# zcablii/SM3Det

Measured on NVIDIA H100. Metric: backbone images/sec @1024^2 (fwd+bwd), higher is better.
Workload: dtype f32 (bf16 hi+lo split operands on wgmma, fp32 accumulate; SIMT fp32 elsewhere)

## Files before the change

include/sm3det_b200.h:

```cpp
#ifndef SM3DET_B200_H_
#define SM3DET_B200_H_

#include <stddef.h>
#include <stdint.h>

#ifdef __cplusplus
extern "C" {
#endif

#define SM3_ABI_VERSION 1

#define SM3_OK 0
#define SM3_ERR_INVALID_ARG (-1)
#define SM3_ERR_UNSUPPORTED_SHAPE (-2)
#define SM3_ERR_CUDA (-3)
#define SM3_ERR_WORKSPACE (-4)

int sm3_abi_version(void);
const char* sm3_last_error(void);
int sm3_device_supported(void);

enum { SM3_SCHED_DENSE = 0, SM3_SCHED_GROUPED = 1, SM3_SCHED_SPLITK = 2 };
enum {
  SM3_EPI_BIAS = 1,
  SM3_EPI_GELU = 2,
  SM3_EPI_DGELU = 4,
  SM3_EPI_COLSCALE = 8,
  SM3_EPI_ROWSCALE = 16,
  SM3_EPI_RESID = 32,
  SM3_EPI_ATOMIC = 64,
  SM3_EPI_AUXSTORE = 128,
  SM3_EPI_COLSUM = 256
};
typedef struct sm3_gemm_args {
  const float* A; int64_t a_stride_mn, a_stride_k;
  const float* B; int64_t b_stride_mn, b_stride_k, b_group_stride;
  const int32_t* a_row_index;
  const int32_t* b_k_index;
  const uint16_t* b_packed;
  int64_t b_packed_group_stride;
  const uint16_t* a_packed;
  int32_t M, N, K;
  int32_t tile_n;
  int32_t sched;
  int32_t k_splits, num_groups;
  const int32_t* tile_group;
  const int32_t* num_m_tiles;
  const int32_t* seg_begin;
  const int32_t* seg_end;
  float* D; int64_t ldd, d_group_stride;
  const float* bias; int64_t bias_group_stride;
  int32_t epilogue;
  float* aux_out; const float* aux_in; int64_t ld_aux;
  const float* col_scale; const float* row_scale;
  const float* resid; int64_t ld_resid;
  float* colsum; int64_t colsum_group_stride;
  int32_t mma_passes;
} sm3_gemm_args;
int sm3_gemm(const sm3_gemm_args* args, void* stream);
int64_t sm3_gemm_packed_elems(int32_t N, int32_t K);
int sm3_gemm_pack_b(const float* B, int64_t stride_mn, int64_t stride_k, int64_t group_stride, int32_t groups,
                    int32_t N, int32_t K, uint16_t* out, void* stream);
int64_t sm3_gemm_packed_act_elems(int64_t rows, int32_t cols, int32_t mn_major, int32_t tile);
int sm3_gemm_pack_act(const float* X, int64_t ld, const int32_t* row_index, int64_t rows, int32_t cols,
                      int32_t mn_major, int32_t tile, uint16_t* out, void* stream);
int32_t sm3_gemm_tile_n(int32_t N);
int sm3_gemm_pack_b_tile(const float* B, int64_t stride_mn, int64_t stride_k, int64_t group_stride, int32_t groups,
                         int32_t N, int32_t K, int32_t tile, uint16_t* out, void* stream);
size_t sm3_gemm_workspace_bytes(const sm3_gemm_args* args);

typedef struct sm3_ffn_args {
  const uint16_t* a1; const uint16_t* a2;
  const uint16_t* wa1; const uint16_t* wa2; const uint16_t* wb;
  const float* bias1;
  const float* bias2;
  const float* col_scale;
  const float* row_scale;
  const float* resid;
  float* out;
  float* aux_out;
  float* h_out;
  int32_t M, C, H4, chunk, mma_passes, mode;
} sm3_ffn_args;
int32_t sm3_ffn_fused_chunk(int32_t mode, int32_t C);
int sm3_ffn_fused(const sm3_ffn_args* args, void* stream);
size_t sm3_ffn_fused_workspace_bytes(const sm3_ffn_args* args);

enum { SM3_LN_NHWC = 0, SM3_LN_PATCH2 = 1, SM3_LN_NCHW = 2 };
int sm3_layernorm_fwd(const float* x, const float* weight, const float* bias, float* y, float* stats,
                      int64_t tokens, int32_t C, float eps, int32_t out_mode, int32_t H, int32_t W, void* stream);
int sm3_layernorm_fwd_img(const float* x, const float* weight, const float* bias, uint16_t* img, float* y, float* stats,
                          int64_t T, int32_t C, float eps, void* stream);
int sm3_layernorm_bwd(const float* dy, const float* x, const float* stats, const float* weight, float* dx,
                      float* dweight, float* dbias, int64_t tokens, int32_t C, int32_t in_mode, int32_t H,
                      int32_t W, int32_t dx_accumulate, void* stream);

int sm3_stem_fwd(const float* x_nchw, const float* weight_t, const float* bias, const float* ln_weight,
                 const float* ln_bias, float* y, float* conv_out, float* stats, int32_t N, int32_t Cin,
                 int32_t H, int32_t W, int32_t ps, int32_t C0, float eps, void* stream);
int sm3_stem_wgrad(const float* x_nchw, const float* dconv, float* dweight_t, float* dbias, int32_t N,
                   int32_t Cin, int32_t H, int32_t W, int32_t ps, int32_t C0, void* stream);

int sm3_dwconv7_fwd(const float* x, const float* weight_t, const float* bias, const float* resid, float* y,
                    int32_t N, int32_t H, int32_t W, int32_t C, void* stream);
int sm3_dwconv7_wgrad(const float* x, const float* dy, float* dweight_t, float* dbias, int32_t N, int32_t H,
                      int32_t W, int32_t C, void* stream);

typedef struct sm3_router_args {
  const float* v; const float* proj_weight; const float* proj_bias; const float* sim_matrix;
  const float* temperature; const float* w_noise; const float* noise;
  int32_t T, C, P, E, k;
  int32_t* top_idx; float* top_gate; float* logits; float* top_vals; float* p_out;
  float* sigma; int32_t* top_idx_m;
  float* partials;
} sm3_router_args;
int sm3_moe_router_blocks(int32_t T);
int sm3_moe_router(const sm3_router_args* args, void* stream);
size_t sm3_moe_router_workspace_bytes(const sm3_router_args* args);

typedef struct sm3_plan_args {
  const float* partials; int32_t T, E, k, max_m_tiles;
  float* importance; float* load; float* loss;
  int32_t* counts; int32_t* seg_begin; int32_t* seg_end; int32_t* cursor;
  int32_t* tile_group; int32_t* num_m_tiles;
} sm3_plan_args;
int sm3_moe_plan(const sm3_plan_args* args, void* stream);
size_t sm3_moe_plan_workspace_bytes(const sm3_plan_args* args);
int sm3_moe_assign(const int32_t* top_idx, int32_t T, int32_t k, int32_t E, const int32_t* seg_begin,
                   int32_t* cursor, int32_t* slot_of, int32_t* pair_token, void* stream);
int sm3_moe_combine(const float* expert_out, const int32_t* slot_of, const int32_t* top_idx, const float* gate,
                    const float* gamma, const float* resid, const float* row_scale, float* out, float* y_opt,
                    int32_t T, int32_t C, int32_t k, void* stream);

typedef struct sm3_act_pack_args {
  const float* h; const float* da; int64_t R; int32_t W; int32_t mode;
  const int32_t* live_tiles; const int32_t* tile_group;
  float* out_f32; uint16_t* pack_k; uint16_t* pack_mn; int32_t mn_tile; float* colsum;
  uint16_t* pack_mn2; int32_t mn_tile2;
} sm3_act_pack_args;
int sm3_act_pack(const sm3_act_pack_args* args, void* stream);

int sm3_moe_combine_bwd(const float* dout, const float* expert_out, const int32_t* slot_of, const int32_t* top_idx,
                        const float* gate, const float* gamma, const float* row_scale, float* d_expert_out,
                        float* dgate, float* dgamma, int32_t T, int32_t C, int32_t k, void* stream);
typedef struct sm3_router_bwd_args {
  const float* p; const float* sim_matrix; const float* temperature;
  const int32_t* top_idx; const float* top_gate; const float* dgate; const float* logits;
  const float* importance; const float* loss_scale;
  int32_t T, P, E, k;
  float* dp; float* dsim_hat; float* dtemperature;
  const float* noise; const float* sigma; const float* top_vals; const int32_t* top_idx_m; const float* load;
  float* dr;
} sm3_router_bwd_args;
int sm3_moe_router_bwd(const sm3_router_bwd_args* args, void* stream);
int sm3_moe_router_bwd_finalize(const float* dsim_hat, const float* sim_matrix, float* dsim, int32_t P, int32_t E,
                                void* stream);
int sm3_colsum(const float* a, const float* b, const float* row_scale, const int32_t* seg_begin,
               const int32_t* seg_end, int32_t groups, float* out, int64_t rows, int32_t C, void* stream);
int sm3_gather_sum(const float* src, const int32_t* slot_of, const float* add, float* out, int32_t T, int32_t C,
                   int32_t k, void* stream);
int sm3_scale_rows(const float* x, const float* row_scale, const float* col_scale, float* out, int64_t rows,
                   int32_t C, void* stream);

int sm3_gather_rows_peer(const float* const* bases, const int32_t* const* token_lists, const int32_t* src_rank,
                         const int32_t* src_row, const float* scale, float* out, int64_t rows, int32_t C, void* stream);

typedef struct sm3_ep_plan_args {
  const int32_t* allm; const int32_t* tile_group_s; const int32_t* num_tiles_s; const int32_t* pair_token;
  int32_t W, me, E, R_s, cap;
  int32_t* src_rank; int32_t* src_slot; int32_t* tile_group; int32_t* num_tiles; int32_t* seg_begin; int32_t* seg_end;
  int32_t* comb_rank; int32_t* comb_row; int32_t* overflow;
} sm3_ep_plan_args;
int sm3_ep_plan(const sm3_ep_plan_args* args, void* stream);

int sm3_dwconv_fwd(const float* x, const float* weight_t, const float* bias, const float* resid, float* y, int32_t N,
                   int32_t H, int32_t W, int32_t C, int32_t ks, int32_t dil, void* stream);
int sm3_dwconv_wgrad(const float* x, const float* dy, float* dweight_t, float* dbias, int32_t N, int32_t H, int32_t W,
                     int32_t C, int32_t ks, int32_t dil, void* stream);
int sm3_colstat(const float* x, const float* sh1, const float* y, const float* sh2, const float* sc2, float* s1, float* s2,
                int64_t rows, int32_t C, void* stream);
int sm3_affine(const float* x1, const float* a1, const float* x2, const float* a2, const float* b, const float* add,
               float* out, int64_t rows, int32_t C, void* stream);
int sm3_mul(const float* a, const float* b, const float* add, float* out, int64_t n, void* stream);
int sm3_dropout(const float* x, float* out, int64_t n, float p, uint64_t seed, void* stream);
int sm3_dropout_dev(const float* x, float* out, int64_t n, float p, const uint64_t* seed_dev, void* stream);
int sm3_lsk_agg(const float* a1, const float* a2, float* agg, int32_t* amax, int64_t T, int32_t Ch, void* stream);
int sm3_conv7_c2(const float* x, const float* w, const float* b, float* y, int32_t N, int32_t H, int32_t W, int32_t act,
                 void* stream);
int sm3_conv7_c2_wgrad(const float* x, const float* dpre, float* dw, float* db, int32_t N, int32_t H, int32_t W, void* stream);
int sm3_lsk_mix(const float* a1, const float* a2, const float* sig, float* out, int64_t T, int32_t Ch, void* stream);
int sm3_lsk_mix_bwd_sig(const float* dout, const float* a1, const float* a2, const float* sig, float* dpre, int64_t T,
                        int32_t Ch, void* stream);
int sm3_lsk_mix_bwd_in(const float* dout, const float* sig, const float* dagg, const int32_t* amax, float* da1, float* da2,
                       int64_t T, int32_t Ch, void* stream);
int sm3_im2col(const float* x, float* col, int32_t N, int32_t H, int32_t W, int32_t Cin, int32_t ks, int32_t stride,
               int32_t pad, int32_t Kp, int32_t nchw, void* stream);
int sm3_col2im(const float* dcol, float* dx, int32_t N, int32_t H, int32_t W, int32_t Cin, int32_t ks, int32_t stride,
               int32_t pad, int32_t Kp, int32_t nchw, void* stream);

int sm3_upsample_add(const float* a, const float* b, float* out, int32_t N, int32_t H, int32_t W, int32_t h, int32_t w,
                     int32_t C, void* stream);
int sm3_upsample_add_bwd(const float* d, float* db, int32_t N, int32_t H, int32_t W, int32_t h, int32_t w, int32_t C,
                         void* stream);
int sm3_transpose_batched(const float* in, float* out, int32_t B, int32_t R, int32_t Cc, void* stream);

#ifdef __cplusplus
}
#endif
#endif
```

sm3det_b200/_lib.py:

```python
import ctypes as C
import os
import threading

_LIB_PATH = os.path.join(os.path.dirname(os.path.abspath(__file__)), 'lib', 'libsm3det_b200.so')
_lock = threading.Lock()
_lib = None
LAUNCHES = 0

c_f32p = C.c_void_p
c_i32p = C.c_void_p
c_stream = C.c_void_p


class GemmArgs(C.Structure):
    _fields_ = [
        ('A', c_f32p), ('a_stride_mn', C.c_int64), ('a_stride_k', C.c_int64),
        ('B', c_f32p), ('b_stride_mn', C.c_int64), ('b_stride_k', C.c_int64), ('b_group_stride', C.c_int64),
        ('a_row_index', c_i32p), ('b_k_index', c_i32p), ('b_packed', C.c_void_p), ('b_packed_group_stride', C.c_int64), ('a_packed', C.c_void_p),
        ('M', C.c_int32), ('N', C.c_int32), ('K', C.c_int32),
        ('tile_n', C.c_int32), ('sched', C.c_int32), ('k_splits', C.c_int32), ('num_groups', C.c_int32),
        ('tile_group', c_i32p), ('num_m_tiles', c_i32p), ('seg_begin', c_i32p), ('seg_end', c_i32p),
        ('D', c_f32p), ('ldd', C.c_int64), ('d_group_stride', C.c_int64),
        ('bias', c_f32p), ('bias_group_stride', C.c_int64),
        ('epilogue', C.c_int32),
        ('aux_out', c_f32p), ('aux_in', c_f32p), ('ld_aux', C.c_int64),
        ('col_scale', c_f32p), ('row_scale', c_f32p),
        ('resid', c_f32p), ('ld_resid', C.c_int64),
        ('colsum', c_f32p), ('colsum_group_stride', C.c_int64),
        ('mma_passes', C.c_int32),
    ]


class RouterArgs(C.Structure):
    _fields_ = [
        ('v', c_f32p), ('proj_weight', c_f32p), ('proj_bias', c_f32p), ('sim_matrix', c_f32p),
        ('temperature', c_f32p), ('w_noise', c_f32p), ('noise', c_f32p),
        ('T', C.c_int32), ('C', C.c_int32), ('P', C.c_int32), ('E', C.c_int32), ('k', C.c_int32),
        ('top_idx', c_i32p), ('top_gate', c_f32p), ('logits', c_f32p), ('top_vals', c_f32p), ('p_out', c_f32p),
        ('sigma', c_f32p), ('top_idx_m', c_i32p),
        ('partials', c_f32p),
    ]


class PlanArgs(C.Structure):
    _fields_ = [
        ('partials', c_f32p), ('T', C.c_int32), ('E', C.c_int32), ('k', C.c_int32), ('max_m_tiles', C.c_int32),
        ('importance', c_f32p), ('load', c_f32p), ('loss', c_f32p),
        ('counts', c_i32p), ('seg_begin', c_i32p), ('seg_end', c_i32p), ('cursor', c_i32p),
        ('tile_group', c_i32p), ('num_m_tiles', c_i32p),
    ]


class FfnArgs(C.Structure):
    _fields_ = [
        ('a1', C.c_void_p), ('a2', C.c_void_p), ('wa1', C.c_void_p), ('wa2', C.c_void_p), ('wb', C.c_void_p),
        ('bias1', c_f32p), ('bias2', c_f32p), ('col_scale', c_f32p), ('row_scale', c_f32p), ('resid', c_f32p),
        ('out', c_f32p), ('aux_out', c_f32p), ('h_out', c_f32p),
        ('M', C.c_int32), ('C', C.c_int32), ('H4', C.c_int32), ('chunk', C.c_int32), ('mma_passes', C.c_int32),
        ('mode', C.c_int32),
    ]


class EpPlanArgs(C.Structure):
    _fields_ = [
        ('allm', c_i32p), ('tile_group_s', c_i32p), ('num_tiles_s', c_i32p), ('pair_token', c_i32p),
        ('W', C.c_int32), ('me', C.c_int32), ('E', C.c_int32), ('R_s', C.c_int32), ('cap', C.c_int32),
        ('src_rank', c_i32p), ('src_slot', c_i32p), ('tile_group', c_i32p), ('num_tiles', c_i32p),
        ('seg_begin', c_i32p), ('seg_end', c_i32p), ('comb_rank', c_i32p), ('comb_row', c_i32p), ('overflow', c_i32p),
    ]


_I32, _I64, _F32, _P = C.c_int32, C.c_int64, C.c_float, C.c_void_p
SIGNATURES = {
    'sm3_abi_version': [],
    'sm3_last_error': [],
    'sm3_device_supported': [],
    'sm3_gemm': [C.POINTER(GemmArgs), _P],
    'sm3_gemm_packed_elems': [_I32, _I32],
    'sm3_gemm_pack_b': [_P, _I64, _I64, _I64, _I32, _I32, _I32, _P, _P],
    'sm3_gemm_packed_act_elems': [_I64, _I32, _I32, _I32],
    'sm3_gemm_pack_act': [_P, _I64, _P, _I64, _I32, _I32, _I32, _P, _P],
    'sm3_gemm_tile_n': [_I32],
    'sm3_gemm_pack_b_tile': [_P, _I64, _I64, _I64, _I32, _I32, _I32, _I32, _P, _P],
    'sm3_gemm_workspace_bytes': [C.POINTER(GemmArgs)],
    'sm3_ffn_fused_chunk': [_I32, _I32],
    'sm3_ffn_fused': [C.POINTER(FfnArgs), _P],
    'sm3_ffn_fused_workspace_bytes': [C.POINTER(FfnArgs)],
    'sm3_moe_router_workspace_bytes': [C.POINTER(RouterArgs)],
    'sm3_moe_plan_workspace_bytes': [C.POINTER(PlanArgs)],
    'sm3_layernorm_fwd': [_P, _P, _P, _P, _P, _I64, _I32, _F32, _I32, _I32, _I32, _P],
    'sm3_layernorm_fwd_img': [_P, _P, _P, _P, _P, _P, _I64, _I32, _F32, _P],
    'sm3_layernorm_bwd': [_P, _P, _P, _P, _P, _P, _P, _I64, _I32, _I32, _I32, _I32, _I32, _P],
    'sm3_stem_fwd': [_P, _P, _P, _P, _P, _P, _P, _P, _I32, _I32, _I32, _I32, _I32, _I32, _F32, _P],
    'sm3_stem_wgrad': [_P, _P, _P, _P, _I32, _I32, _I32, _I32, _I32, _I32, _P],
    'sm3_dwconv7_fwd': [_P, _P, _P, _P, _P, _I32, _I32, _I32, _I32, _P],
    'sm3_dwconv7_wgrad': [_P, _P, _P, _P, _I32, _I32, _I32, _I32, _P],
    'sm3_moe_router_bwd_finalize': [_P, _P, _P, _I32, _I32, _P],
    'sm3_moe_router_blocks': [_I32],
    'sm3_moe_router': [C.POINTER(RouterArgs), _P],
    'sm3_moe_plan': [C.POINTER(PlanArgs), _P],
    'sm3_moe_assign': [_P, _I32, _I32, _I32, _P, _P, _P, _P, _P],
    'sm3_moe_combine': [_P, _P, _P, _P, _P, _P, _P, _P, _P, _I32, _I32, _I32, _P],
    'sm3_moe_combine_bwd': [_P, _P, _P, _P, _P, _P, _P, _P, _P, _P, _I32, _I32, _I32, _P],
    'sm3_colsum': [_P, _P, _P, _P, _P, _I32, _P, _I64, _I32, _P],
    'sm3_gather_sum': [_P, _P, _P, _P, _I32, _I32, _I32, _P],
    'sm3_scale_rows': [_P, _P, _P, _P, _I64, _I32, _P],
    'sm3_moe_router_bwd': [_P, _P],
    'sm3_ep_plan': [C.POINTER(EpPlanArgs), _P],
    'sm3_gather_rows_peer': [_P, _P, _P, _P, _P, _P, _I64, _I32, _P],
    'sm3_upsample_add': [_P, _P, _P, _I32, _I32, _I32, _I32, _I32, _I32, _P],
    'sm3_upsample_add_bwd': [_P, _P, _I32, _I32, _I32, _I32, _I32, _I32, _P],
    'sm3_transpose_batched': [_P, _P, _I32, _I32, _I32, _P],
    'sm3_dwconv_fwd': [_P, _P, _P, _P, _P, _I32, _I32, _I32, _I32, _I32, _I32, _P],
    'sm3_dwconv_wgrad': [_P, _P, _P, _P, _I32, _I32, _I32, _I32, _I32, _I32, _P],
    'sm3_colstat': [_P, _P, _P, _P, _P, _P, _P, _I64, _I32, _P],
    'sm3_affine': [_P, _P, _P, _P, _P, _P, _P, _I64, _I32, _P],
    'sm3_mul': [_P, _P, _P, _P, _I64, _P],
    'sm3_dropout': [_P, _P, _I64, _F32, C.c_uint64, _P],
    'sm3_dropout_dev': [_P, _P, _I64, _F32, _P, _P],
    'sm3_lsk_agg': [_P, _P, _P, _P, _I64, _I32, _P],
    'sm3_conv7_c2': [_P, _P, _P, _P, _I32, _I32, _I32, _I32, _P],
    'sm3_conv7_c2_wgrad': [_P, _P, _P, _P, _I32, _I32, _I32, _P],
    'sm3_lsk_mix': [_P, _P, _P, _P, _I64, _I32, _P],
    'sm3_lsk_mix_bwd_sig': [_P, _P, _P, _P, _P, _I64, _I32, _P],
    'sm3_lsk_mix_bwd_in': [_P, _P, _P, _P, _P, _P, _I64, _I32, _P],
    'sm3_im2col': [_P, _P, _I32, _I32, _I32, _I32, _I32, _I32, _I32, _I32, _I32, _P],
    'sm3_col2im': [_P, _P, _I32, _I32, _I32, _I32, _I32, _I32, _I32, _I32, _I32, _P],
}
_RESTYPES = {'sm3_last_error': C.c_char_p, 'sm3_gemm_packed_elems': C.c_int64, 'sm3_gemm_packed_act_elems': C.c_int64,
             'sm3_gemm_workspace_bytes': C.c_size_t, 'sm3_ffn_fused_workspace_bytes': C.c_size_t,
             'sm3_moe_router_workspace_bytes': C.c_size_t, 'sm3_moe_plan_workspace_bytes': C.c_size_t}


class ActPackArgs(C.Structure):
    _fields_ = [
        ('h', c_f32p), ('da', c_f32p), ('R', C.c_int64), ('W', C.c_int32), ('mode', C.c_int32),
        ('live_tiles', c_i32p), ('tile_group', c_i32p),
        ('out_f32', c_f32p), ('pack_k', C.c_void_p), ('pack_mn', C.c_void_p), ('mn_tile', C.c_int32), ('colsum', c_f32p),
        ('pack_mn2', C.c_void_p), ('mn_tile2', C.c_int32),
    ]


class RouterBwdArgs(C.Structure):
    _fields_ = [
        ('p', c_f32p), ('sim_matrix', c_f32p), ('temperature', c_f32p),
        ('top_idx', c_i32p), ('top_gate', c_f32p), ('dgate', c_f32p), ('logits', c_f32p),
        ('importance', c_f32p), ('loss_scale', c_f32p),
        ('T', C.c_int32), ('P', C.c_int32), ('E', C.c_int32), ('k', C.c_int32),
        ('dp', c_f32p), ('dsim_hat', c_f32p), ('dtemperature', c_f32p),
        ('noise', c_f32p), ('sigma', c_f32p), ('top_vals', c_f32p), ('top_idx_m', c_i32p), ('load', c_f32p),
        ('dr', c_f32p),
    ]


SIGNATURES['sm3_moe_router_bwd'] = [C.POINTER(RouterBwdArgs), _P]
SIGNATURES['sm3_act_pack'] = [C.POINTER(ActPackArgs), _P]


def library_path() -> str:
    return _LIB_PATH


def load():
    global _lib
    if _lib is not None:
        return _lib
    with _lock:
        if _lib is not None:
            return _lib
        if not os.path.isfile(_LIB_PATH):
            raise RuntimeError(
                f'sm3det_b200: CUDA library not built ({_LIB_PATH} missing). Run `make` at the repo root or '
                f'`python -c "import __graft_entry__ as g; g.build()"`. There is no CPU/PyTorch fallback.')
        lib = C.CDLL(_LIB_PATH)
        for name, argtypes in SIGNATURES.items():
            fn = getattr(lib, name)
            fn.argtypes = argtypes
            fn.restype = _RESTYPES.get(name, C.c_int)
        if lib.sm3_abi_version() != 1:
            raise RuntimeError('sm3det_b200: ABI version mismatch')
        _lib = lib
    return _lib


def check(rc: int, what: str):
    global LAUNCHES
    LAUNCHES += 1
    if rc != 0:
        msg = load().sm3_last_error()
        raise RuntimeError(f'sm3det_b200: {what} failed (rc={rc}): {msg.decode() if msg else "?"}')
```

sm3det_b200/backbone.py:

```python
import math
from typing import Sequence

import torch
import torch.nn as nn

from . import functional as Fn
from .registry import ROTATED_BACKBONES, BaseModule

ARCH_SETTINGS = {
    'atto': dict(depths=[2, 2, 6, 2], channels=[40, 80, 160, 320]),
    'femto': dict(depths=[2, 2, 6, 2], channels=[48, 96, 192, 384]),
    'pico': dict(depths=[2, 2, 6, 2], channels=[64, 128, 256, 512]),
    'nano': dict(depths=[2, 2, 8, 2], channels=[80, 160, 320, 640]),
    'tiny': dict(depths=[3, 3, 9, 3], channels=[96, 192, 384, 768]),
    'small': dict(depths=[3, 3, 27, 3], channels=[96, 192, 384, 768]),
    'base': dict(depths=[3, 3, 27, 3], channels=[128, 256, 512, 1024]),
    'swin_large': dict(depths=[2, 2, 18, 2], channels=[192, 384, 768, 1536]),
    'large': dict(depths=[3, 3, 27, 3], channels=[192, 384, 768, 1536]),
    'xlarge': dict(depths=[3, 3, 27, 3], channels=[256, 512, 1024, 2048]),
    'huge': dict(depths=[3, 3, 27, 3], channels=[352, 704, 1408, 2816]),
}


class LayerNorm2d(nn.LayerNorm):

    def __init__(self, num_channels: int, **kwargs) -> None:
        super().__init__(num_channels, **kwargs)
        self.num_channels = self.normalized_shape[0]


def build_LayerNorm2d_layer(cfg: dict, num_features: int) -> nn.Module:
    if not isinstance(cfg, dict):
        raise TypeError('cfg must be a dict')
    if 'type' not in cfg:
        raise KeyError('the cfg dict must contain the key "type"')
    cfg_ = cfg.copy()
    cfg_.pop('type')
    requires_grad = cfg_.pop('requires_grad', True)
    cfg_.setdefault('eps', 1e-5)
    layer = LayerNorm2d(num_features, **cfg_)
    for param in layer.parameters():
        param.requires_grad = requires_grad
    return layer


class FFN(nn.Module):
    def __init__(self, in_channels, mid_channels):
        super().__init__()
        self.pointwise_conv1 = nn.Linear(in_channels, mid_channels)
        self.pointwise_conv2 = nn.Linear(mid_channels, in_channels)


class CosineTopKGate(nn.Module):
    def __init__(self, model_dim, num_global_experts, init_t=0.5):
        super().__init__()
        proj_dim = min(model_dim // 2, 256)
        self.temperature = nn.Parameter(torch.log(torch.full([1], 1.0 / init_t)), requires_grad=True)
        self.cosine_projector = nn.Linear(model_dim, proj_dim)
        self.sim_matrix = nn.Parameter(torch.randn(size=(proj_dim, num_global_experts)), requires_grad=True)
        nn.init.normal_(self.sim_matrix, 0, 0.01)


class MoE_layer(nn.Module):
    def __init__(self, in_channels, mid_channels, num_experts, top_k, noisy_gating, gating):
        super().__init__()
        if gating != 'cosine':
            raise NotImplementedError(
                "sm3det_b200: only gate='cosine' is implemented (gate='linear' starts from an all-zero w_gate, "
                'i.e. fully tied logits whose routing is implementation-defined in the reference)')
        assert top_k <= num_experts
        self.noisy_gating = noisy_gating
        self.num_experts = num_experts
        self.input_size = in_channels
        self.k = top_k
        self.gating = gating
        self.experts = nn.ModuleList([FFN(in_channels, mid_channels) for _ in range(num_experts)])
        self.w_gate = CosineTopKGate(in_channels, num_experts)
        self.w_noise = nn.Parameter(torch.zeros(in_channels, num_experts), requires_grad=True)
        self.register_buffer('mean', torch.tensor([0.0]))
        self.register_buffer('std', torch.tensor([1.0]))

    def expert_params(self):
        e = self.experts
        w1 = [m.pointwise_conv1.weight for m in e]
        b1 = [m.pointwise_conv1.bias for m in e]
        w2 = [m.pointwise_conv2.weight for m in e]
        b2 = [m.pointwise_conv2.bias for m in e]
        for group in (w1, b1, w2, b2):
            Fn.stack_expert_params(group)
        return w1 + b1 + w2 + b2


class PackCache:

    def __init__(self):
        self._d = {}

    def invalidate(self):
        self._d.clear()

    def get(self, name, params, transposed, tile=0):
        from . import ops
        key = tuple(p._version for p in params) + (params[0].data_ptr(), str(params[0].device))
        name = (name, tile)
        hit = self._d.get((name, transposed))
        if hit is not None and hit[0] == key:
            return hit[1]
        reuse = None if hit is None or hit[1][0].device != params[0].device else hit[1][0]
        with torch.no_grad():
            packed = ops.pack_weight(params[0], transposed=transposed, groups=len(params), out=reuse, tile=tile)
        self._d[(name, transposed)] = (key, packed)
        return packed


class ConvNeXtBlock(nn.Module):
    def __init__(self, in_channels, norm_cfg, mlp_ratio=4., MoE_cfg=None, drop_path_rate=0.,
                 layer_scale_init_value=1e-6):
        super().__init__()
        self.depthwise_conv = nn.Conv2d(in_channels, in_channels, groups=in_channels, kernel_size=7, padding=3)
        self.norm = build_LayerNorm2d_layer(norm_cfg, in_channels)
        mid = int(mlp_ratio * in_channels)
        self.MoE_cfg = MoE_cfg
        if MoE_cfg is not None:
            self.ffn = MoE_layer(in_channels, mid, MoE_cfg['num_experts'], MoE_cfg['top_k'], MoE_cfg['noisy_gating'],
                                 MoE_cfg['gating'])
        else:
            self.ffn = FFN(in_channels, mid)
        if not layer_scale_init_value > 0:
            raise NotImplementedError('sm3det_b200: layer_scale_init_value must be > 0 (gamma is fused in the epilogue)')
        self.gamma = nn.Parameter(layer_scale_init_value * torch.ones((in_channels)), requires_grad=True)
        self.drop_path_rate = float(drop_path_rate)
        self._packs = PackCache()

    def _apply(self, fn, recurse=True):
        self._packs.invalidate()
        return super()._apply(fn, recurse)

    def _load_from_state_dict(self, *args, **kwargs):
        self._packs.invalidate()
        return super()._load_from_state_dict(*args, **kwargs)

    def _row_scale(self, x):
        if self.drop_path_rate == 0. or not self.training:
            return None
        keep = 1.0 - self.drop_path_rate
        N, H, W, _ = x.shape
        mask = getattr(self, '_injected_drop_mask', None)
        if mask is None:
            mask = x.new_empty((N,)).bernoulli_(keep)
            if keep > 0.0:
                mask = mask / keep
        return mask.to(x.device, torch.float32).repeat_interleave(H * W).contiguous()

    def forward(self, x, record=None):
        return self._run(x, self._row_scale(x), record, True)

    def _run(self, x, rs, record, shortcut):
        eps = self.norm.eps
        dw = self.depthwise_conv
        grad = torch.is_grad_enabled()
        pc = self._packs
        from . import ops
        if self.MoE_cfg is None:
            f = self.ffn
            w1, w2 = f.pointwise_conv1.weight, f.pointwise_conv2.weight
            C = w2.shape[0]
            cf = ops.ffn_chunk(0, C)
            if cf > 0:
                packs = {'fused': dict(fwd=cf), 'w1_c': pc.get('w1', [w1], False, tile=cf), 'w2_n': pc.get('w2', [w2], False, tile=C)}
            else:
                packs = {'w1': pc.get('w1', [w1], False), 'w2': pc.get('w2', [w2], False)}
            if grad:
                packs['w1_t'] = pc.get('w1', [w1], True)
            packs['grad'] = grad
            packs['shortcut'] = shortcut
            out = Fn.DenseBlockFn.apply(x, dw.weight, dw.bias, self.norm.weight, self.norm.bias,
                                        w1, f.pointwise_conv1.bias, w2, f.pointwise_conv2.bias, self.gamma, rs, eps, packs)
            return out, None
        m = self.ffn
        noise = None
        if m.noisy_gating and self.training:
            noise = getattr(m, '_injected_noise', None)
            if noise is None:
                T = x.shape[0] * x.shape[1] * x.shape[2]
                noise = torch.randn((T, m.num_experts), device=x.device, dtype=torch.float32)
            noise = noise.to(x.device, torch.float32).contiguous()
        g = m.w_gate
        ep = m.expert_params()
        E = m.num_experts
        w1s, w2s = ep[0:E], ep[2 * E:3 * E]
        epc = getattr(self, '_ep', None)
        if epc is not None:
            if not shortcut:
                raise NotImplementedError('sm3det_b200: expert parallelism is not wired for the ConvNeXt_DA blocks')
            from .expert_parallel import EPMoEBlockFn
            El = E // epc.world
            o1, o2 = w1s[epc.rank * El:(epc.rank + 1) * El], w2s[epc.rank * El:(epc.rank + 1) * El]
            packs = {'w1': pc.get('w1', o1, False), 'w2': pc.get('w2', o2, False)}
            if grad:
                packs['w1_t'] = pc.get('w1', o1, True)
                packs['w2_t'] = pc.get('w2', o2, True)
                packs['wp_t'] = pc.get('wp', [g.cosine_projector.weight], True)
            return EPMoEBlockFn.apply(x, dw.weight, dw.bias, self.norm.weight, self.norm.bias, self.gamma,
                                      g.cosine_projector.weight, g.cosine_projector.bias, g.sim_matrix, g.temperature,
                                      m.w_noise, rs, noise, eps, E, m.k, record, packs, epc, self._ep_key, *ep)
        packs = {'w1': pc.get('w1', w1s, False), 'w2': pc.get('w2', w2s, False)}
        if grad:
            packs['w1_t'] = pc.get('w1', w1s, True)
            packs['w2_t'] = pc.get('w2', w2s, True)
            packs['wp_t'] = pc.get('wp', [g.cosine_projector.weight], True)
        packs['shortcut'] = shortcut
        out, loss = Fn.MoEBlockFn.apply(x, dw.weight, dw.bias, self.norm.weight, self.norm.bias, self.gamma,
                                        g.cosine_projector.weight, g.cosine_projector.bias, g.sim_matrix, g.temperature,
                                        m.w_noise, rs, noise, eps, E, m.k, record, packs, *ep)
        return out, loss


class DALayer(nn.Module):
    dataset_DA = {'sar': 0, 'rgb': 1, 'ifr': 2}

    def __init__(self, channel, reduction=16):
        super().__init__()
        self.avg_pool = nn.AdaptiveAvgPool2d(1)
        self.fc = nn.ModuleList([nn.Sequential(nn.Linear(channel, channel // reduction, bias=False), nn.ReLU(inplace=True),
                                               nn.Linear(channel // reduction, channel, bias=False), nn.Sigmoid())] * 3)

    def gate(self, m, datasets):
        with torch.autocast('cuda', enabled=False):
            if len(datasets) == 1:
                return self.fc[self.dataset_DA[datasets[0]]](m)
            if len(datasets) != m.shape[0]:
                raise ValueError(f'ConvNeXt_DA: {len(datasets)} dataset names for a batch of {m.shape[0]} (the reference zips them '
                                 f'sample by sample, convnext_moe_DA.py:315-318)')
            return torch.cat([self.fc[self.dataset_DA[d]](row.view(1, -1)) for row, d in zip(m, datasets)], dim=0)


class ConvNeXtDABlock(ConvNeXtBlock):

    def __init__(self, *args, **kwargs):
        super().__init__(*args, **kwargs)
        self.avg_pool = nn.AdaptiveAvgPool2d(1)
        self.DA = DALayer(self.gamma.shape[0])

    def forward(self, x, record=None, datasets=('rgb',)):
        rs = self._row_scale(x)
        y, loss = self._run(x, None, record, False)
        s = self.DA.gate(Fn.SampleMeanFn.apply(y), list(datasets))
        return Fn.DAGateFn.apply(y, x, s, rs), loss


@ROTATED_BACKBONES.register_module()
class ConvNeXt_moe(BaseModule):
    arch_settings = ARCH_SETTINGS
    block_cls = ConvNeXtBlock

    def __init__(self, arch='tiny', in_channels=3, stem_patch_size=4, norm_cfg=dict(type='LN2d', eps=1e-6),
                 act_cfg=dict(type='GELU'), linear_pw_conv=True, use_grn=False, drop_path_rate=0.,
                 layer_scale_init_value=1e-6, out_indices=[0, 1, 2, 3], MoE_Block_inds=[[], [], [], []],
                 noisy_gating=True, num_experts=2, gate='cosine', top_k=2, frozen_stages=0,
                 gap_before_final_norm=False, with_cp=False,
                 init_cfg=[dict(type='TruncNormal', layer=['Conv2d', 'Linear'], std=.02, bias=0.),
                           dict(type='Constant', layer=['LayerNorm'], val=1., bias=0.)]):
        super().__init__(init_cfg=init_cfg)
        if isinstance(arch, str):
            assert arch in self.arch_settings, \
                f'Unavailable arch, please choose from ({set(self.arch_settings)}) or pass a dict.'
            arch = self.arch_settings[arch]
        elif isinstance(arch, dict):
            assert 'depths' in arch and 'channels' in arch, \
                f'The arch dict must have "depths" and "channels", but got {list(arch.keys())}.'
        if act_cfg.get('type', 'GELU') != 'GELU':
            raise NotImplementedError('sm3det_b200: only act_cfg=dict(type="GELU") is implemented')
        if not linear_pw_conv:
            raise NotImplementedError('sm3det_b200: linear_pw_conv=False (1x1 Conv2d FFN) is not implemented')
        if use_grn:
            raise NotImplementedError('sm3det_b200: use_grn=True is not implemented (no SM3Det config enables it)')
        if gap_before_final_norm:
            raise NotImplementedError('sm3det_b200: gap_before_final_norm=True is not implemented')
        self.depths = list(arch['depths'])
        self.channels = list(arch['channels'])
        assert (isinstance(self.depths, Sequence) and isinstance(self.channels, Sequence)
                and len(self.depths) == len(self.channels))
        for c in self.channels:
            if c % 32 != 0 or c > 1024:
                raise NotImplementedError(f'sm3det_b200: channel count {c} unsupported (multiple of 32, <= 1024)')
        self.num_stages = len(self.depths)
        if isinstance(out_indices, int):
            out_indices = [out_indices]
        out_indices = list(out_indices)
        for i, index in enumerate(out_indices):
            if index < 0:
                out_indices[i] = 4 + index
                assert out_indices[i] >= 0, f'Invalid out_indices {index}'
        self.out_indices = out_indices
        self.MoE_Block_inds = MoE_Block_inds
        self.num_experts = num_experts
        self.frozen_stages = frozen_stages
        self.gap_before_final_norm = gap_before_final_norm
        self.with_cp = with_cp
        self.stem_patch_size = stem_patch_size
        self.norm_eps = norm_cfg.get('eps', 1e-5)

        dpr = [x.item() for x in torch.linspace(0, drop_path_rate, sum(self.depths), device='cpu')]
        block_idx = 0
        self.downsample_layers = nn.ModuleList()
        stem = nn.Sequential(
            nn.Conv2d(in_channels, self.channels[0], kernel_size=stem_patch_size, stride=stem_patch_size),
            build_LayerNorm2d_layer(norm_cfg, self.channels[0]))
        self.downsample_layers.append(stem)
        self.stages = nn.ModuleList()
        for i in range(self.num_stages):
            depth = self.depths[i]
            channels = self.channels[i]
            if i >= 1:
                self.downsample_layers.append(nn.Sequential(
                    build_LayerNorm2d_layer(norm_cfg, self.channels[i - 1]),
                    nn.Conv2d(self.channels[i - 1], channels, kernel_size=2, stride=2)))
            moe_ind = [list(range(depth))[q] for q in self.MoE_Block_inds[i] if q < depth]
            stage = nn.Sequential(*[
                self.block_cls(in_channels=channels, drop_path_rate=dpr[block_idx + j], norm_cfg=norm_cfg,
                              MoE_cfg={'noisy_gating': noisy_gating, 'num_experts': num_experts, 'top_k': top_k,
                                       'gating': gate} if j in moe_ind else None,
                              layer_scale_init_value=layer_scale_init_value) for j in range(depth)])
            block_idx += depth
            self.stages.append(stage)
            if i in self.out_indices:
                self.add_module(f'norm{i}', build_LayerNorm2d_layer(norm_cfg, channels))
        self._init_like_reference()
        self._freeze_stages()

    def _init_like_reference(self):
        """The reference never runs init_cfg (init_weights() only supports 'Pretrained'); weights stay at
        torch defaults.  We keep torch's default constructors too, so nothing to do."""

    def _stem(self, x):
        conv, ln = self.downsample_layers[0][0], self.downsample_layers[0][1]
        return Fn.StemFn.apply(x, conv.weight, conv.bias, ln.weight, ln.bias, ln.eps, self.stem_patch_size)

    def _trunk(self, x, record=None, datasets=None):
        outs, gate_losses = [], []
        for i, stage in enumerate(self.stages):
            if i >= 1:
                ln, conv = self.downsample_layers[i][0], self.downsample_layers[i][1]
                x = Fn.DownsampleFn.apply(x, ln.weight, ln.bias, conv.weight, conv.bias, ln.eps)
            for blk in stage:
                x, gate_loss = blk(x, record) if datasets is None else blk(x, record, datasets)
                if gate_loss is not None:
                    gate_losses.append(gate_loss)
            if i in self.out_indices:
                nl = getattr(self, f'norm{i}')
                outs.append(Fn.OutNormFn.apply(x, nl.weight, nl.bias, nl.eps))
        if len(gate_losses) > 0:
            return tuple(outs), sum(gate_losses) / len(gate_losses)
        return tuple(outs)

    def forward(self, x, record=None):
        self._check_input(x)
        with self._precision():
            return self._trunk(self._stem(x), record)

    def _precision(self):
        from . import ops
        return ops.precision_scope(ops.autocast_passes(self))

    @staticmethod
    def _check_input(x):
        if not x.is_cuda:
            raise RuntimeError('sm3det_b200 backbones run on CUDA (sm_90a) only; there is no CPU path')
        if x.dim() != 4 or x.shape[2] % 32 != 0 or x.shape[3] % 32 != 0:
            raise ValueError(f'expected [N,3,H,W] with H, W multiples of 32 (Pad size_divisor=32), got {tuple(x.shape)}')

    def _freeze_stages(self):
        for i in range(self.frozen_stages):
            downsample_layer = self.downsample_layers[i]
            stage = self.stages[i]
            downsample_layer.eval()
            stage.eval()
            for param in list(downsample_layer.parameters()) + list(stage.parameters()):
                param.requires_grad = False

    def train(self, mode=True):
        super().train(mode)
        self._freeze_stages()
        return self

    def get_layer_depth(self, param_name: str, prefix: str = ''):
        max_layer_id = 12 if self.depths[-2] > 9 else 6
        if not param_name.startswith(prefix):
            return max_layer_id + 1, max_layer_id + 2
        param_name = param_name[len(prefix):]
        if param_name.startswith('downsample_layers'):
            stage_id = int(param_name.split('.')[1])
            if stage_id == 0:
                layer_id = 0
            elif stage_id == 1 or stage_id == 2:
                layer_id = stage_id + 1
            else:
                layer_id = max_layer_id
        elif param_name.startswith('stages'):
            stage_id = int(param_name.split('.')[1])
            block_id = int(param_name.split('.')[2])
            if stage_id == 0 or stage_id == 1:
                layer_id = stage_id + 1
            elif stage_id == 2:
                layer_id = 3 + block_id // 3
            else:
                layer_id = max_layer_id
        else:
            layer_id = max_layer_id + 1
        return layer_id, max_layer_id + 2

    def upcycle_state_dict(self, src, multi_input=False):
        out = {}
        for k, v in src.items():
            if not k.startswith('backbone.'):
                continue
            k = k[9:]
            if multi_input and 'downsample_layers.0.0' in k:
                out[k.replace('downsample_layers.0.0', 'dataset_stems.single')] = v
            elif multi_input and 'downsample_layers.0.1' in k:
                out[k.replace('downsample_layers.0.1', 'downsample_layers.0.0')] = v
            elif 'pointwise_conv' in k:
                parts = k.split('.')
                stage_ind, block_ind = int(parts[1]), int(parts[2])
                if block_ind in self.MoE_Block_inds[stage_ind]:
                    for e in range(self.num_experts):
                        out[k.replace('pointwise_conv', f'ffn.experts.{e}.pointwise_conv')] = v
                else:
                    out[k.replace('pointwise_conv', 'ffn.pointwise_conv')] = v
            else:
                out[k] = v
        if out and next(iter(out)).startswith('module.'):
            out = {k[7:]: v for k, v in out.items()}
        return out

    def init_weights(self):
        cfg = self.init_cfg
        if isinstance(cfg, dict) and cfg.get('type') == 'Pretrained' and cfg.get('checkpoint'):
            ckpt = torch.load(cfg['checkpoint'], map_location='cpu')
            sd = ckpt.get('state_dict', ckpt.get('model', ckpt))
            sd = self.upcycle_state_dict(sd, multi_input=isinstance(self, ConvNeXt_moe_MultiInput))
            print(self.load_state_dict(sd, strict=False))


@ROTATED_BACKBONES.register_module()
class ConvNeXt_moe_MultiInput(ConvNeXt_moe):
    def __init__(self, arch='tiny', in_channels=3, stem_patch_size=4, datasets=None,
                 norm_cfg=dict(type='LN2d', eps=1e-6), act_cfg=dict(type='GELU'), linear_pw_conv=True,
                 use_grn=False, drop_path_rate=0., layer_scale_init_value=1e-6, out_indices=[0, 1, 2, 3],
                 MoE_Block_inds=[[], [], [], []], noisy_gating=True, num_experts=2, top_k=2, gate='cosine',
                 frozen_stages=0, gap_before_final_norm=False, with_cp=False,
                 init_cfg=[dict(type='TruncNormal', layer=['Conv2d', 'Linear'], std=.02, bias=0.),
                           dict(type='Constant', layer=['LayerNorm'], val=1., bias=0.)]):
        super().__init__(MoE_Block_inds=MoE_Block_inds, noisy_gating=noisy_gating, num_experts=num_experts,
                         gate=gate, top_k=top_k, arch=arch, in_channels=in_channels,
                         stem_patch_size=stem_patch_size, norm_cfg=norm_cfg, act_cfg=act_cfg,
                         linear_pw_conv=linear_pw_conv, use_grn=use_grn, drop_path_rate=drop_path_rate,
                         layer_scale_init_value=layer_scale_init_value, out_indices=out_indices,
                         frozen_stages=frozen_stages, gap_before_final_norm=gap_before_final_norm,
                         with_cp=with_cp, init_cfg=init_cfg)
        self.downsample_layers[0] = nn.Sequential(build_LayerNorm2d_layer(norm_cfg, self.channels[0]))
        self.datasets = ['single']
        self.dataset_stems = nn.ModuleDict()
        self.dataset_stems['single'] = nn.Conv2d(in_channels, self.channels[0], kernel_size=stem_patch_size,
                                                 stride=stem_patch_size)

    def _stem(self, x):
        conv, ln = self.dataset_stems['single'], self.downsample_layers[0][0]
        return Fn.StemFn.apply(x, conv.weight, conv.bias, ln.weight, ln.bias, ln.eps, self.stem_patch_size)

    def forward(self, x, datasets=['single'], record=None):
        if len(datasets) == 1:
            x = [x]
        x = torch.cat(list(x), dim=0)
        self._check_input(x)
        with self._precision():
            return self._trunk(self._stem(x), record)


@ROTATED_BACKBONES.register_module()
class ConvNeXt_DA_MultiInput(ConvNeXt_moe_MultiInput):
    block_cls = ConvNeXtDABlock

    def __init__(self, *args, datasets=None, **kwargs):
        super().__init__(*args, datasets=datasets, **kwargs)
        if datasets is not None and list(datasets) != ['single']:
            raise NotImplementedError('sm3det_b200: per-dataset stems (datasets=[...]) are not implemented; the reference forward '
                                      "only ever uses dataset_stems['single'] (convnext_moe_DA.py:836)")
        self.init_datasets = datasets

    def forward(self, x, datasets=['single'], record=None):
        if len(datasets) == 1:
            x = [x]
        x = torch.cat(list(x), dim=0)
        self._check_input(x)
        with self._precision():
            return self._trunk(self._stem(x), record, list(datasets))

    def init_weights(self):
        super().init_weights()
        cfg = self.init_cfg
        if isinstance(cfg, dict) and cfg.get('type') == 'Pretrained':
            for stage in self.stages:
                for blk in stage:
                    for m in range(3):
                        nn.init.constant_(blk.DA.fc[m][2].weight, 0.0)
```

sm3det_b200/csrc/capi.cu:

```cuda
#include "../../include/sm3det_b200.h"
#include "common.cuh"
#include "gemm_tc.cuh"
#include "kernels.h"
#include "ffn_fused.cuh"

using namespace sm3;

static inline cudaStream_t S(void* s) { return reinterpret_cast<cudaStream_t>(s); }

extern "C" {

int sm3_abi_version(void) { return SM3_ABI_VERSION; }
const char* sm3_last_error(void) { return sm3::last_error(); }

int sm3_device_supported(void) {
  int dev = 0, major = 0, minor = 0;
  if (cudaGetDevice(&dev) != cudaSuccess) return 0;
  if (cudaDeviceGetAttribute(&major, cudaDevAttrComputeCapabilityMajor, dev) != cudaSuccess) return 0;
  if (cudaDeviceGetAttribute(&minor, cudaDevAttrComputeCapabilityMinor, dev) != cudaSuccess) return 0;
  return (major == 9 && minor == 0) ? 1 : 0;
}

int sm3_gemm(const sm3_gemm_args* a, void* stream) {
  if (!a) { set_last_error("sm3_gemm: null args"); return SM3_ERR_INVALID_ARG; }
  gemm::Params p{};
  p.A = a->A; p.a_smn = a->a_stride_mn; p.a_sk = a->a_stride_k;
  p.B = a->B; p.b_smn = a->b_stride_mn; p.b_sk = a->b_stride_k; p.b_group_stride = a->b_group_stride;
  p.a_row_index = a->a_row_index; p.b_k_index = a->b_k_index;
  p.b_packed = a->b_packed; p.b_packed_group_stride = a->b_packed_group_stride; p.a_packed = a->a_packed;
  p.M = a->M; p.N = a->N; p.K = a->K; p.BN = a->tile_n;
  p.sched = a->sched; p.k_splits = a->k_splits; p.num_groups = a->num_groups;
  p.tile_group = a->tile_group; p.num_m_tiles_dev = a->num_m_tiles;
  p.seg_begin = a->seg_begin; p.seg_end = a->seg_end;
  p.D = a->D; p.ldd = a->ldd; p.d_group_stride = a->d_group_stride;
  p.bias = a->bias; p.bias_group_stride = a->bias_group_stride;
  p.epi = a->epilogue;
  p.aux_out = a->aux_out; p.aux_in = a->aux_in; p.ld_aux = a->ld_aux;
  p.col_scale = a->col_scale; p.row_scale = a->row_scale;
  p.resid = a->resid; p.ld_resid = a->ld_resid;
  p.colsum = a->colsum; p.colsum_group_stride = a->colsum_group_stride;
  p.passes = (a->mma_passes == 1) ? 1 : 3;
  return gemm::launch(p, S(stream));
}

int64_t sm3_gemm_packed_elems(int32_t N, int32_t K) { return gemm::packed_elems(N, K); }
int sm3_gemm_pack_b(const float* B, int64_t s_mn, int64_t s_k, int64_t group_stride, int32_t groups, int32_t N, int32_t K,
                    uint16_t* out, void* stream) {
  return gemm::pack_b(B, s_mn, s_k, group_stride, groups, N, K, out, S(stream));
}

int64_t sm3_gemm_packed_act_elems(int64_t rows, int32_t cols, int32_t mn_major, int32_t tile) {
  return gemm::packed_act_elems(rows, cols, mn_major, tile);
}
int sm3_gemm_pack_act(const float* X, int64_t ld, const int32_t* row_index, int64_t rows, int32_t cols, int32_t mn_major,
                      int32_t tile, uint16_t* out, void* stream) {
  return gemm::pack_act(X, ld, row_index, rows, cols, mn_major, tile, out, S(stream));
}
int32_t sm3_gemm_tile_n(int32_t N) { return gemm::pick_bn(N); }
int sm3_gemm_pack_b_tile(const float* B, int64_t s_mn, int64_t s_k, int64_t group_stride, int32_t groups, int32_t N, int32_t K,
                         int32_t tile, uint16_t* out, void* stream) {
  return gemm::pack_b(B, s_mn, s_k, group_stride, groups, N, K, out, S(stream), tile);
}
size_t sm3_gemm_workspace_bytes(const sm3_gemm_args*) { return 0; }

int32_t sm3_ffn_fused_chunk(int32_t mode, int32_t C) { return (mode == 0 || mode == 1) ? ffn::chain_chunk(mode, C) : 0; }
size_t sm3_ffn_fused_workspace_bytes(const sm3_ffn_args*) { return 0; }
int sm3_ffn_fused(const sm3_ffn_args* a, void* stream) {
  if (!a) { set_last_error("sm3_ffn_fused: null args"); return SM3_ERR_INVALID_ARG; }
  ffn::ChainParams p{};
  p.a1 = a->a1; p.a2 = a->a2; p.wa1 = a->wa1; p.wa2 = a->wa2; p.wb = a->wb;
  p.bias1 = a->bias1; p.bias2 = a->bias2; p.col_scale = a->col_scale; p.row_scale = a->row_scale; p.resid = a->resid;
  p.out = a->out; p.aux_out = a->aux_out; p.h_out = a->h_out;
  p.M = a->M; p.C = a->C; p.H4 = a->H4; p.HC = a->chunk; p.passes = a->mma_passes; p.mode = a->mode;
  return ffn::chain(p, S(stream));
}

int sm3_layernorm_fwd(const float* x, const float* w, const float* b, float* y, float* stats, int64_t T, int32_t C,
                      float eps, int32_t out_mode, int32_t H, int32_t W, void* stream) {
  return layernorm_fwd(x, w, b, y, stats, T, C, eps, out_mode, H, W, S(stream));
}
int sm3_layernorm_fwd_img(const float* x, const float* w, const float* b, uint16_t* img, float* y, float* stats, int64_t T,
                          int32_t C, float eps, void* stream) {
  return layernorm_fwd_img(x, w, b, img, y, stats, T, C, eps, S(stream));
}
int sm3_layernorm_bwd(const float* dy, const float* x, const float* stats, const float* w, float* dx, float* dw,
                      float* db, int64_t T, int32_t C, int32_t in_mode, int32_t H, int32_t W, int32_t dx_accum,
                      void* stream) {
  return layernorm_bwd(dy, x, stats, w, dx, dw, db, T, C, in_mode, H, W, dx_accum, S(stream));
}
int sm3_stem_fwd(const float* x, const float* wt, const float* bias, const float* lnw, const float* lnb, float* y,
                 float* conv_out, float* stats, int32_t N, int32_t Cin, int32_t H, int32_t W, int32_t ps, int32_t C0,
                 float eps, void* stream) {
  return stem_fwd(x, wt, bias, lnw, lnb, y, conv_out, stats, N, Cin, H, W, ps, C0, eps, S(stream));
}
int sm3_stem_wgrad(const float* x, const float* du, float* dwt, float* dbias, int32_t N, int32_t Cin, int32_t H,
                   int32_t W, int32_t ps, int32_t C0, void* stream) {
  return stem_wgrad(x, du, dwt, dbias, N, Cin, H, W, ps, C0, S(stream));
}
int sm3_dwconv7_fwd(const float* x, const float* wt, const float* bias, const float* resid, float* y, int32_t N,
                    int32_t H, int32_t W, int32_t C, void* stream) {
  return dwconv7_fwd(x, wt, bias, resid, y, N, H, W, C, S(stream));
}
int sm3_dwconv7_wgrad(const float* x, const float* dy, float* dwt, float* dbias, int32_t N, int32_t H, int32_t W,
                      int32_t C, void* stream) {
  return dwconv7_wgrad(x, dy, dwt, dbias, N, H, W, C, S(stream));
}

int sm3_moe_router_blocks(int32_t T) { return router_blocks(T); }
int sm3_moe_router(const sm3_router_args* a, void* stream) {
  if (!a) { set_last_error("sm3_moe_router: null args"); return SM3_ERR_INVALID_ARG; }
  RouterArgs r{};
  r.v = a->v; r.wp = a->proj_weight; r.bp = a->proj_bias; r.sim = a->sim_matrix; r.temperature = a->temperature;
  r.w_noise = a->w_noise; r.noise = a->noise;
  r.T = a->T; r.C = a->C; r.P = a->P; r.E = a->E; r.k = a->k;
  r.top_idx = a->top_idx; r.top_gate = a->top_gate; r.logits = a->logits; r.top_vals = a->top_vals; r.p_out = a->p_out; r.sigma = a->sigma; r.top_idx_m = a->top_idx_m;
  r.partials = a->partials; r.nblocks = router_blocks(a->T);
  return moe_router(r, S(stream));
}
size_t sm3_moe_router_workspace_bytes(const sm3_router_args* a) {
  return a ? (size_t)router_blocks(a->T) * 3u * (size_t)a->E * sizeof(float) : 0;
}
size_t sm3_moe_plan_workspace_bytes(const sm3_plan_args* a) {
  return a ? (size_t)(2 * a->E + 1) * sizeof(float) + (size_t)(4 * a->E + a->max_m_tiles + 1) * sizeof(int32_t) : 0;
}
int sm3_moe_plan(const sm3_plan_args* a, void* stream) {
  if (!a) { set_last_error("sm3_moe_plan: null args"); return SM3_ERR_INVALID_ARG; }
  PlanArgs p{};
  p.partials = a->partials; p.nblocks = router_blocks(a->T);
  p.T = a->T; p.E = a->E; p.k = a->k; p.max_m_tiles = a->max_m_tiles;
  p.importance = a->importance; p.load = a->load; p.loss = a->loss;
  p.counts = a->counts; p.seg_begin = a->seg_begin; p.seg_end = a->seg_end; p.cursor = a->cursor;
  p.tile_group = a->tile_group; p.num_m_tiles = a->num_m_tiles;
  return moe_plan(p, S(stream));
}
int sm3_moe_assign(const int32_t* top_idx, int32_t T, int32_t k, int32_t E, const int32_t* seg_begin, int32_t* cursor,
                   int32_t* slot_of, int32_t* pair_token, void* stream) {
  return moe_assign(top_idx, T, k, E, seg_begin, cursor, slot_of, pair_token, S(stream));
}
int sm3_moe_combine(const float* o, const int32_t* slot_of, const int32_t* top_idx, const float* gate,
                    const float* gamma, const float* resid, const float* row_scale, float* out, float* y_opt,
                    int32_t T, int32_t C, int32_t k, void* stream) {
  return moe_combine(o, slot_of, top_idx, gate, gamma, resid, row_scale, out, y_opt, T, C, k, S(stream));
}

int sm3_act_pack(const sm3_act_pack_args* a, void* stream) {
  if (!a) { set_last_error("sm3_act_pack: null args"); return SM3_ERR_INVALID_ARG; }
  ActPackArgs r{};
  r.h = a->h; r.da = a->da; r.R = a->R; r.W = a->W; r.mode = a->mode; r.live_tiles = a->live_tiles; r.tile_group = a->tile_group;
  r.out_f32 = a->out_f32; r.pack_k = a->pack_k; r.pack_mn = a->pack_mn; r.mn_tile = a->mn_tile; r.colsum = a->colsum;
  r.pack_mn2 = a->pack_mn2; r.mn_tile2 = a->mn_tile2;
  return act_pack(r, S(stream));
}
int sm3_moe_combine_bwd(const float* dout, const float* o, const int32_t* slot_of, const int32_t* top_idx,
                        const float* gate, const float* gamma, const float* row_scale, float* d_o, float* dgate,
                        float* dgamma, int32_t T, int32_t C, int32_t k, void* stream) {
  return moe_combine_bwd(dout, o, slot_of, top_idx, gate, gamma, row_scale, d_o, dgate, dgamma, T, C, k, S(stream));
}
int sm3_moe_router_bwd(const sm3_router_bwd_args* a, void* stream) {
  if (!a) { set_last_error("sm3_moe_router_bwd: null args"); return SM3_ERR_INVALID_ARG; }
  RouterBwdArgs r{};
  r.p = a->p; r.sim = a->sim_matrix; r.temperature = a->temperature; r.top_idx = a->top_idx; r.top_gate = a->top_gate;
  r.dgate = a->dgate; r.logits = a->logits; r.importance = a->importance; r.loss_scale = a->loss_scale;
  r.T = a->T; r.P = a->P; r.E = a->E; r.k = a->k; r.dp = a->dp; r.dsim_hat = a->dsim_hat; r.dtemperature = a->dtemperature;
  r.noise = a->noise; r.sigma = a->sigma; r.top_vals = a->top_vals; r.top_idx_m = a->top_idx_m; r.load = a->load; r.dr = a->dr;
  return moe_router_bwd(r, S(stream));
}
int sm3_moe_router_bwd_finalize(const float* dsim_hat, const float* sim, float* dsim, int32_t P, int32_t E, void* stream) {
  return moe_router_bwd_finalize(dsim_hat, sim, dsim, P, E, S(stream));
}
int sm3_colsum(const float* a, const float* b, const float* rs, const int32_t* seg_begin, const int32_t* seg_end,
               int32_t G, float* out, int64_t rows, int32_t C, void* stream) {
  return colsum(a, b, rs, seg_begin, seg_end, G, out, rows, C, S(stream));
}
int sm3_gather_sum(const float* src, const int32_t* slot_of, const float* add, float* out, int32_t T, int32_t C,
                   int32_t k, void* stream) {
  return gather_sum(src, slot_of, add, out, T, C, k, S(stream));
}
int sm3_scale_rows(const float* x, const float* rs, const float* cs, float* out, int64_t rows, int32_t C, void* stream) {
  return scale_rows(x, rs, cs, out, rows, C, S(stream));
}

int sm3_gather_rows_peer(const float* const* bases, const int32_t* const* token_lists, const int32_t* src_rank,
                         const int32_t* src_row, const float* scale, float* out, int64_t rows, int32_t C, void* stream) {
  return gather_rows_peer(bases, reinterpret_cast<const int* const*>(token_lists), src_rank, src_row, scale, out, rows, C, S(stream));
}
int sm3_dwconv_fwd(const float* x, const float* wt, const float* bias, const float* resid, float* y, int32_t N, int32_t H,
                   int32_t W, int32_t C, int32_t ks, int32_t dil, void* stream) {
  return dwconv_fwd(x, wt, bias, resid, y, N, H, W, C, ks, dil, S(stream));
}
int sm3_dwconv_wgrad(const float* x, const float* dy, float* dwt, float* dbias, int32_t N, int32_t H, int32_t W, int32_t C,
                     int32_t ks, int32_t dil, void* stream) {
  return dwconv_wgrad(x, dy, dwt, dbias, N, H, W, C, ks, dil, S(stream));
}
int sm3_colstat(const float* x, const float* sh1, const float* y, const float* sh2, const float* sc2, float* s1, float* s2,
                int64_t rows, int32_t C, void* stream) {
  return colstat(x, sh1, y, sh2, sc2, s1, s2, rows, C, S(stream));
}
int sm3_affine(const float* x1, const float* a1, const float* x2, const float* a2, const float* b, const float* add,
               float* out, int64_t rows, int32_t C, void* stream) {
  return affine(x1, a1, x2, a2, b, add, out, rows, C, S(stream));
}
int sm3_mul(const float* a, const float* b, const float* add, float* out, int64_t n, void* stream) {
  return mul(a, b, add, out, n, S(stream));
}
int sm3_dropout(const float* x, float* out, int64_t n, float p, uint64_t seed, void* stream) {
  return dropout(x, out, n, p, seed, S(stream));
}
int sm3_dropout_dev(const float* x, float* out, int64_t n, float p, const uint64_t* seed_dev, void* stream) {
  return dropout_dev(x, out, n, p, reinterpret_cast<const unsigned long long*>(seed_dev), S(stream));
}
int sm3_lsk_agg(const float* a1, const float* a2, float* agg, int32_t* amax, int64_t T, int32_t Ch, void* stream) {
  return lsk_agg(a1, a2, agg, amax, T, Ch, S(stream));
}
int sm3_conv7_c2(const float* x, const float* w, const float* b, float* y, int32_t N, int32_t H, int32_t W, int32_t act,
                 void* stream) {
  return conv7_c2(x, w, b, y, N, H, W, act, S(stream));
}
int sm3_conv7_c2_wgrad(const float* x, const float* dpre, float* dw, float* db, int32_t N, int32_t H, int32_t W, void* stream) {
  return conv7_c2_wgrad(x, dpre, dw, db, N, H, W, S(stream));
}
int sm3_lsk_mix(const float* a1, const float* a2, const float* sig, float* out, int64_t T, int32_t Ch, void* stream) {
  return lsk_mix(a1, a2, sig, out, T, Ch, S(stream));
}
int sm3_lsk_mix_bwd_sig(const float* dout, const float* a1, const float* a2, const float* sig, float* dpre, int64_t T,
                        int32_t Ch, void* stream) {
  return lsk_mix_bwd_sig(dout, a1, a2, sig, dpre, T, Ch, S(stream));
}
int sm3_lsk_mix_bwd_in(const float* dout, const float* sig, const float* dagg, const int32_t* amax, float* da1, float* da2,
                       int64_t T, int32_t Ch, void* stream) {
  return lsk_mix_bwd_in(dout, sig, dagg, amax, da1, da2, T, Ch, S(stream));
}
int sm3_im2col(const float* x, float* col, int32_t N, int32_t H, int32_t W, int32_t Cin, int32_t ks, int32_t stride,
               int32_t pad, int32_t Kp, int32_t nchw, void* stream) {
  return im2col(x, col, N, H, W, Cin, ks, stride, pad, Kp, nchw, S(stream));
}
int sm3_col2im(const float* dcol, float* dx, int32_t N, int32_t H, int32_t W, int32_t Cin, int32_t ks, int32_t stride,
               int32_t pad, int32_t Kp, int32_t nchw, void* stream) {
  return col2im(dcol, dx, N, H, W, Cin, ks, stride, pad, Kp, nchw, S(stream));
}

int sm3_ep_plan(const sm3_ep_plan_args* a, void* stream) {
  if (!a) { set_last_error("sm3_ep_plan: null args"); return SM3_ERR_INVALID_ARG; }
  EpPlanArgs p{};
  p.allm = a->allm; p.tile_group_s = a->tile_group_s; p.num_tiles_s = a->num_tiles_s; p.pair_token = a->pair_token;
  p.W = a->W; p.me = a->me; p.E = a->E; p.R_s = a->R_s; p.cap = a->cap;
  p.src_rank = a->src_rank; p.src_slot = a->src_slot; p.tile_group = a->tile_group; p.num_tiles = a->num_tiles;
  p.seg_begin = a->seg_begin; p.seg_end = a->seg_end; p.comb_rank = a->comb_rank; p.comb_row = a->comb_row; p.overflow = a->overflow;
  return ep_plan(p, S(stream));
}

int sm3_upsample_add(const float* a, const float* b, float* out, int32_t N, int32_t H, int32_t W, int32_t h, int32_t w,
                     int32_t C, void* stream) {
  return upsample_add(a, b, out, N, H, W, h, w, C, S(stream));
}
int sm3_upsample_add_bwd(const float* d, float* db, int32_t N, int32_t H, int32_t W, int32_t h, int32_t w, int32_t C,
                         void* stream) {
  return upsample_add_bwd(d, db, N, H, W, h, w, C, S(stream));
}
int sm3_transpose_batched(const float* in, float* out, int32_t B, int32_t R, int32_t Cc, void* stream) {
  return transpose_batched(in, out, B, R, Cc, S(stream));
}

}
```

sm3det_b200/csrc/ffn_fused.cu:

```cuda
#define SM3_GEMM_KERNEL_IMPL
#include "gemm_tc.cuh"
#include "ffn_fused.cuh"
#include "kernels.h"

namespace sm3 {
namespace ffn {
using namespace gemm;

constexpr int THREADS = 384;
constexpr int W_PROD_A = 0, W_PROD_B = 1, EPI0 = 4, NE = 8;
constexpr int CONS_REGS = 232, PROD_REGS = 40;
constexpr uint32_t SMEM_LIMIT = 232448u - 1024u;
constexpr uint32_t STAGING = NE * EPI_STAGE_BYTES;
constexpr uint32_t BARS = 256;

struct Layout {
  uint32_t a, ones, a2, wa, wb, act, act2, stage, bar, total;
  uint32_t a_tile, wa_chunk, wa_stage, wb_stage, act_bytes;
  int sa, sb;
};

struct ChainK { ChainParams p; Layout L; int m_tiles, nch; };

__device__ __forceinline__ void bulk_g2s(uint32_t dst, const void* src, uint32_t bytes, uint32_t bar) {
  asm volatile("cp.async.bulk.shared::cluster.global.mbarrier::complete_tx::bytes [%0], [%1], %2, [%3];"
               ::"r"(dst), "l"(src), "r"(bytes), "r"(bar) : "memory");
}
__device__ __forceinline__ void expect_tx(uint32_t bar, uint32_t bytes) {
  asm volatile("mbarrier.arrive.expect_tx.shared::cta.b64 _, [%0], %1;" ::"r"(bar), "r"(bytes) : "memory");
}
__device__ __forceinline__ void sts128(uint32_t addr, uint32_t a, uint32_t b, uint32_t c, uint32_t d) {
  asm volatile("st.shared.v4.b32 [%0], {%1, %2, %3, %4};" ::"r"(addr), "r"(a), "r"(b), "r"(c), "r"(d) : "memory");
}

__device__ __forceinline__ void split2(float v0, float v1, uint32_t& hi, uint32_t& lo) {
  const uint32_t u0 = __float_as_uint(v0), u1 = __float_as_uint(v1);
  hi = __byte_perm(u0, u1, 0x7632);
  const uint32_t r0 = __float_as_uint(v0 - __uint_as_float(u0 & 0xFFFF0000u)) + 0x8000u;
  const uint32_t r1 = __float_as_uint(v1 - __uint_as_float(u1 & 0xFFFF0000u)) + 0x8000u;
  lo = __byte_perm(r0, r1, 0x7632);
}

template <int N, int NA>
__device__ __forceinline__ void mma3(float (&d)[NA], uint64_t ahi, uint64_t alo, uint64_t bhi, uint64_t blo, uint32_t accum,
                                     int passes) {
  if (passes == 1) {
    wg::mma<N, 0, 0>(d, ahi, bhi, accum);
  } else {
    wg::mma<N, 0, 0>(d, alo, bhi, accum);
    wg::mma<N, 0, 0>(d, ahi, blo, 1u);
    wg::mma<N, 0, 0>(d, ahi, bhi, 1u);
  }
}

template <int MODE, int HC, int C>
__global__ void __launch_bounds__(THREADS, 1) ffn_chain_kernel(const __grid_constant__ ChainK k) {
  const ChainParams& p = k.p;
  const Layout& L = k.L;
  extern __shared__ uint8_t smem_raw[];
  const uint32_t sb0 = (smem_u32(smem_raw) + 1023u) & ~1023u;
  const uint32_t bar = sb0 + L.bar;
  const uint32_t a_full = bar, a_empty = bar + 8;
  auto wa_full = [&](int s) { return bar + 16u + 8u * s; };
  auto wa_empty = [&](int s) { return bar + 32u + 8u * s; };
  auto wb_full = [&](int s) { return bar + 48u + 8u * s; };
  auto wb_empty = [&](int s) { return bar + 64u + 8u * s; };
  const int warp = threadIdx.x >> 5, lane = threadIdx.x & 31;
  constexpr int NA = (MODE == 1) ? 2 : 1;

  if (threadIdx.x == 0) {
    mbar_init(a_full, 1); mbar_init(a_empty, NE);
    for (int s = 0; s < 2; ++s) { mbar_init(wa_full(s), 1); mbar_init(wa_empty(s), NE); mbar_init(wb_full(s), 1); mbar_init(wb_empty(s), NE); }
    asm volatile("fence.mbarrier_init.release.cluster;" ::: "memory");
  }
  __syncthreads();
  const int nch = k.nch;
  constexpr int kbc = C / 32;

  if (warp < EPI0) {
    asm volatile("setmaxnreg.dec.sync.aligned.u32 %0;" ::"n"(PROD_REGS));
    if (warp == W_PROD_A && lane == 0) {
      uint32_t n_t = 0, n_w = 0;
      for (int t = blockIdx.x; t < k.m_tiles; t += gridDim.x, ++n_t) {
        mbar_wait(a_empty, (n_t & 1u) ^ 1u);
        if ((p.debug & 8) && n_t > 0) { mbar_arrive(a_full); goto weights; }
        expect_tx(a_full, NA * L.a_tile);
        bulk_g2s(sb0 + L.a, reinterpret_cast<const uint8_t*>(p.a1) + (long long)t * L.a_tile, L.a_tile, a_full);
        if (MODE == 1) bulk_g2s(sb0 + L.a + L.a_tile, reinterpret_cast<const uint8_t*>(p.a2) + (long long)t * L.a_tile, L.a_tile, a_full);
      weights:
        for (int j = 0; j < nch; ++j, ++n_w) {
          const int s = n_w % L.sa;
          mbar_wait(wa_empty(s), ((n_w / L.sa) & 1u) ^ 1u);
          if ((p.debug & 4) && n_w >= (uint32_t)L.sa) { mbar_arrive(wa_full(s)); continue; }
          expect_tx(wa_full(s), L.wa_stage);
          const uint32_t dst = sb0 + L.wa + s * L.wa_stage;
          bulk_g2s(dst, reinterpret_cast<const uint8_t*>(p.wa1) + (long long)j * L.wa_chunk, L.wa_chunk, wa_full(s));
          if (MODE == 1) bulk_g2s(dst + L.wa_chunk, reinterpret_cast<const uint8_t*>(p.wa2) + (long long)j * L.wa_chunk, L.wa_chunk, wa_full(s));
        }
      }
    } else if (warp == W_PROD_B && lane == 0) {
      uint32_t n = 0;
      for (int t = blockIdx.x; t < k.m_tiles; t += gridDim.x) {
        for (int j = 0; j < nch; ++j, ++n) {
          const int s = n % L.sb;
          mbar_wait(wb_empty(s), ((n / L.sb) & 1u) ^ 1u);
          if ((p.debug & 4) && n >= (uint32_t)L.sb) { mbar_arrive(wb_full(s)); continue; }
          expect_tx(wb_full(s), L.wb_stage);
          bulk_g2s(sb0 + L.wb + s * L.wb_stage, reinterpret_cast<const uint8_t*>(p.wb) + (long long)j * L.wb_stage, L.wb_stage, wb_full(s));
        }
      }
    }
  } else {
    asm volatile("setmaxnreg.inc.sync.aligned.u32 %0;" ::"n"(CONS_REGS));
    const int e = warp - EPI0, g = e >> 2, wq = warp & 3;
    const uint32_t slab = (uint32_t)g * WG_A_BYTES;
    const uint32_t stage_base = sb0 + L.stage + (uint32_t)e * EPI_STAGE_BYTES;
    const int rl = lane >> 2, c4 = (lane & 3) * 4;
    const int r_lo = g * 64 + wq * 16 + rl;
    auto wg_bar = [&]() { asm volatile("bar.sync %0, 128;" ::"r"(1 + g) : "memory"); };
    float acc_h[HC / 2], acc_d[HC / 2], acc_o[C / 2];
    uint32_t n_c = 0, n_b = 0, n_t = 0;
    auto gemm_a = [&](uint32_t nc) {
      const int s = nc % L.sa;
      mbar_wait(wa_full(s), (nc / L.sa) & 1u);
      const uint32_t wst = sb0 + L.wa + s * L.wa_stage;
#pragma unroll
      for (int q = 0; q < NA; ++q) {
        uint64_t da = make_smem_desc(sb0 + L.a + q * L.a_tile + slab, false), db = make_smem_desc(wst + q * L.wa_chunk, false);
        for (int kb = 0; kb < kbc; ++kb) {
          if (q == 0) {
            mma3<HC>(acc_h, da, da + 512u, db, db + HC * 4u, kb > 0 ? 1u : 0u, p.passes);
            mma3<HC>(acc_h, da + 2u, da + 514u, db + 2u, db + HC * 4u + 2u, 1u, p.passes);
          } else {
            mma3<HC>(acc_d, da, da + 512u, db, db + HC * 4u, kb > 0 ? 1u : 0u, p.passes);
            mma3<HC>(acc_d, da + 2u, da + 514u, db + 2u, db + HC * 4u + 2u, 1u, p.passes);
          }
          da += 1024u; db += HC * 8u;
        }
      }
    };
    for (int t = blockIdx.x; t < k.m_tiles; t += gridDim.x, ++n_t) {
      mbar_wait(a_full, n_t & 1u);
      wg::fence();
      gemm_a(n_c);
      wg::commit();
      for (int j = 0; j < nch; ++j, ++n_c) {
        wg::wait<0>();
        wg::fence_operand(acc_h);
        if constexpr (MODE == 1) wg::fence_operand(acc_d);
        __syncwarp();
        if (lane == 0) {
          mbar_arrive(wa_empty(n_c % L.sa));
          if (j > 0) mbar_arrive(wb_empty((n_b - 1) % L.sb));
          if (j == nch - 1) mbar_arrive(a_empty);
        }
        const float* b1 = p.bias1 + (long long)j * HC;
#pragma unroll
        for (int q = 0; q < HC / 8; ++q) {
          const int kk = 8 * q + 2 * (lane & 3);
          const float2 bv = __ldg(reinterpret_cast<const float2*>(b1 + kk));
#pragma unroll
          for (int h = 0; h < 2; ++h) {
            const int r = r_lo + 8 * h;
            const float x0 = acc_h[4 * q + 2 * h] + bv.x, x1 = acc_h[4 * q + 2 * h + 1] + bv.y;
            if (MODE == 0 && p.h_out) {
              const long long row = (long long)t * 128 + r;
              if (row < p.M) *reinterpret_cast<float2*>(p.h_out + row * p.H4 + (long long)j * HC + kk) = make_float2(x0, x1);
            }
            float y0, y1;
            if (p.debug & 1) { y0 = x0; y1 = x1; }
            else if constexpr (MODE == 0) { y0 = gelu_fast(x0); y1 = gelu_fast(x1); }
            else { y0 = acc_d[4 * q + 2 * h] * gelu_grad_fast(x0); y1 = acc_d[4 * q + 2 * h + 1] * gelu_grad_fast(x1); }
            if (p.debug & 2) continue;
            uint32_t hi, lo;
            split2(y0, y1, hi, lo);
            const uint32_t o = sb0 + L.act + (uint32_t)(kk >> 5) * 16384u + kmajor_sw64_offset((uint32_t)r, (uint32_t)((kk & 31) >> 3)) +
                               (uint32_t)(kk & 7) * 2u;
            asm volatile("st.shared.b32 [%0], %1;" ::"r"(o), "r"(hi) : "memory");
            asm volatile("st.shared.b32 [%0], %1;" ::"r"(o + 8192u), "r"(lo) : "memory");
          }
        }
        fence_proxy_async_smem();
        wg_bar();
        const int s = n_b % L.sb;
        mbar_wait(wb_full(s), (n_b / L.sb) & 1u);
        wg::fence();
        {
          uint64_t da = make_smem_desc(sb0 + L.act + slab, false), db = make_smem_desc(sb0 + L.wb + s * L.wb_stage, false);
          const uint64_t blo = (uint64_t)(C * 4);
#pragma unroll
          for (int kb = 0; kb < HC / 32; ++kb) {
            mma3<C>(acc_o, da, da + 512u, db, db + blo, (j > 0 || kb > 0) ? 1u : 0u, p.passes);
            mma3<C>(acc_o, da + 2u, da + 514u, db + 2u, db + blo + 2u, 1u, p.passes);
            da += 1024u; db += 2u * blo;
          }
        }
        ++n_b;
        if (j + 1 < nch) gemm_a(n_c + 1);
        wg::commit();
      }
      wg::wait<0>();
      wg::fence_operand(acc_o);
      __syncwarp();
      if (lane == 0) mbar_arrive(wb_empty((n_b - 1) % L.sb));
      const long long row0 = (long long)t * 128 + g * 64 + wq * 16;
#pragma unroll
      for (int c = 0; c < C / 16; ++c) {
        const int n = c * 16 + c4;
        float4 rr[2];
#pragma unroll
        for (int it = 0; it < 2; ++it) {
          const long long row = row0 + it * 8 + rl;
          rr[it] = (p.resid && row < p.M) ? ldg_f4(p.resid + row * C + n) : make_float4(0.f, 0.f, 0.f, 0.f);
        }
        __syncwarp();
#pragma unroll
        for (int qq = 0; qq < 2; ++qq)
#pragma unroll
          for (int h = 0; h < 2; ++h)
            asm volatile("st.shared.v2.f32 [%0], {%1, %2};"
                         ::"r"(stage_base + (uint32_t)((rl + 8 * h) * EPI_STAGE_ROW_FLOATS + 8 * qq + 2 * (lane & 3)) * 4u),
                           "f"(acc_o[8 * c + 4 * qq + 2 * h]), "f"(acc_o[8 * c + 4 * qq + 2 * h + 1]) : "memory");
        __syncwarp();
        float4 bv = make_float4(0.f, 0.f, 0.f, 0.f), sv = make_float4(1.f, 1.f, 1.f, 1.f);
        if (p.bias2) bv = ldg_f4(p.bias2 + n);
        if (p.col_scale) sv = ldg_f4(p.col_scale + n);
#pragma unroll
        for (int it = 0; it < 2; ++it) {
          const int rr_ = it * 8 + rl;
          const long long row = row0 + rr_;
          if (row >= p.M) continue;
          float4 x;
          asm volatile("ld.shared.v4.f32 {%0, %1, %2, %3}, [%4];" : "=f"(x.x), "=f"(x.y), "=f"(x.z), "=f"(x.w)
                       : "r"(stage_base + (uint32_t)(rr_ * EPI_STAGE_ROW_FLOATS + c4) * 4u) : "memory");
          x.x += bv.x; x.y += bv.y; x.z += bv.z; x.w += bv.w;
          if (p.aux_out) *reinterpret_cast<float4*>(p.aux_out + row * C + n) = x;
          x.x *= sv.x; x.y *= sv.y; x.z *= sv.z; x.w *= sv.w;
          if (p.row_scale) { const float rs = __ldg(p.row_scale + row); x.x *= rs; x.y *= rs; x.z *= rs; x.w *= rs; }
          x.x += rr[it].x; x.y += rr[it].y; x.z += rr[it].z; x.w += rr[it].w;
          *reinterpret_cast<float4*>(p.out + row * C + n) = x;
        }
      }
    }
  }
}

static bool chain_layout(int mode, int C, int HC, int sa, int sb, Layout& L) {
  const uint32_t nA = mode == 1 ? 2 : 1;
  L.a_tile = (uint32_t)(C / 32) * 16384u;
  L.wa_chunk = (uint32_t)(C / 32) * HC * 128u;
  L.wa_stage = nA * L.wa_chunk;
  L.wb_stage = (uint32_t)(HC / 32) * C * 128u;
  L.act_bytes = (uint32_t)(HC / 32) * 16384u;
  L.sa = sa; L.sb = sb;
  uint32_t o = 0;
  L.a = o; o += nA * L.a_tile;
  L.ones = 0; L.a2 = L.a + L.a_tile;
  L.wa = o; o += sa * L.wa_stage;
  L.wb = o; o += sb * L.wb_stage;
  L.act = o; o += L.act_bytes;
  L.act2 = 0;
  L.stage = o; o += STAGING;
  L.bar = o; o += BARS;
  L.total = o + 1024u;
  return L.total <= SMEM_LIMIT + 1024u;
}

static bool pick_chain(int mode, int C, int HC_req, int& HC, Layout& L) {
  static const int cand[][3] = {{64, 2, 2}, {32, 2, 2}, {64, 2, 1}, {32, 2, 1}, {32, 1, 1}};
  if (C % 32 != 0 || C < 32 || C > 256) return false;
  for (auto& c : cand)
    if ((HC_req == 0 || c[0] == HC_req) && chain_layout(mode, C, c[0], c[1], c[2], L)) { HC = c[0]; return true; }
  return false;
}

int chain_chunk(int mode, int C) {
  int HC = 0; Layout L;
  return pick_chain(mode, C, 0, HC, L) ? HC : 0;
}

static bool aligned16(const void* q) { return (reinterpret_cast<uintptr_t>(q) & 15u) == 0; }

int chain(const ChainParams& p, cudaStream_t stream) {
  SM3_REQUIRE(p.mode == 0 || p.mode == 1, SM3_ERR_INVALID_ARG, "ffn chain: mode");
  SM3_REQUIRE(p.a1 && p.wa1 && p.wb && p.bias1 && p.out && (p.mode == 0 || (p.a2 && p.wa2)), SM3_ERR_INVALID_ARG, "ffn chain: null operand");
  SM3_REQUIRE(p.M > 0 && p.H4 > 0 && p.C > 0, SM3_ERR_INVALID_ARG, "ffn chain: bad shape");
  ChainK k{};
  k.p = p;
  int HC = 0;
  SM3_REQUIRE(p.HC == 32 || p.HC == 64, SM3_ERR_INVALID_ARG, "ffn chain: chunk must be 32 or 64 (sm3_ffn_fused_chunk), got %d", p.HC);
  SM3_REQUIRE(pick_chain(p.mode, p.C, p.HC, HC, k.L), SM3_ERR_UNSUPPORTED_SHAPE, "ffn chain: C=%d with chunk %d does not fit shared memory (mode %d)", p.C, p.HC, p.mode);
  SM3_REQUIRE(p.H4 % HC == 0 && p.C % 16 == 0, SM3_ERR_UNSUPPORTED_SHAPE, "ffn chain: H4=%d not a multiple of the chunk %d", p.H4, HC);
  SM3_REQUIRE(aligned16(p.a1) && aligned16(p.wa1) && aligned16(p.wb) && aligned16(p.out) && aligned16(p.bias1) &&
              (!p.a2 || aligned16(p.a2)) && (!p.wa2 || aligned16(p.wa2)) && (!p.resid || aligned16(p.resid)) &&
              (!p.aux_out || aligned16(p.aux_out)) && (!p.bias2 || aligned16(p.bias2)) && (!p.col_scale || aligned16(p.col_scale)),
              SM3_ERR_INVALID_ARG, "ffn chain: pointers must be 16B aligned");
  k.p.passes = (p.passes == 1) ? 1 : 3;
  k.m_tiles = (p.M + 127) / 128;
  k.nch = p.H4 / HC;
  int grid = persistent_grid_sms();
  if (grid > k.m_tiles) grid = k.m_tiles;
#define SM3_CHAIN_LAUNCH(MODE_, HC_, C_)                                                                                    \
  do {                                                                                                                      \
    cudaFuncSetAttribute(ffn_chain_kernel<MODE_, HC_, C_>, cudaFuncAttributeMaxDynamicSharedMemorySize, (int)k.L.total);    \
    ffn_chain_kernel<MODE_, HC_, C_><<<grid, THREADS, k.L.total, stream>>>(k);                                              \
  } while (0)
#define SM3_CHAIN_C(MODE_, HC_)                                                                                             \
  switch (p.C) {                                                                                                            \
    case 32: SM3_CHAIN_LAUNCH(MODE_, HC_, 32); break;   case 64: SM3_CHAIN_LAUNCH(MODE_, HC_, 64); break;                   \
    case 96: SM3_CHAIN_LAUNCH(MODE_, HC_, 96); break;   case 128: SM3_CHAIN_LAUNCH(MODE_, HC_, 128); break;                 \
    case 160: SM3_CHAIN_LAUNCH(MODE_, HC_, 160); break; case 192: SM3_CHAIN_LAUNCH(MODE_, HC_, 192); break;                 \
    case 224: SM3_CHAIN_LAUNCH(MODE_, HC_, 224); break; default: SM3_CHAIN_LAUNCH(MODE_, HC_, 256); break;                  \
  }
  if (p.mode == 0) { if (HC == 64) { SM3_CHAIN_C(0, 64) } else { SM3_CHAIN_C(0, 32) } }
  else { if (HC == 64) { SM3_CHAIN_C(1, 64) } else { SM3_CHAIN_C(1, 32) } }
#undef SM3_CHAIN_C
#undef SM3_CHAIN_LAUNCH
  return check_launch("ffn_chain_kernel");
}

}
}
```

sm3det_b200/csrc/ffn_fused.cuh:

```cuda
#pragma once
#include <cuda_runtime.h>
#include <stdint.h>

namespace sm3 {
namespace ffn {

struct ChainParams {
  const uint16_t* a1;
  const uint16_t* a2;
  const uint16_t* wa1;
  const uint16_t* wa2;
  const uint16_t* wb;
  const float* bias1;
  const float* bias2;
  const float* col_scale;
  const float* row_scale;
  const float* resid;
  float* out;
  float* aux_out;
  float* h_out;
  int M, C, H4, HC, passes, mode;
  int debug;
};
int chain(const ChainParams& p, cudaStream_t stream);

int chain_chunk(int mode, int C);

}
}
```

sm3det_b200/functional.py:

```python
import torch
from torch.autograd import Function

from . import ops
from .ops import (EPI_AUXSTORE, EPI_COLSCALE, EPI_DGELU, EPI_GELU, EPI_RESID, EPI_ROWSCALE, LN_NCHW, LN_NHWC, LN_PATCH2)


def _zeros_like_param(p):
    return torch.zeros(p.shape, device=p.device, dtype=torch.float32)


def _taps(dww):
    return dww.reshape(dww.shape[0], 49).t().contiguous()


def _taps_flipped(dww):
    return dww.flip(2, 3).reshape(dww.shape[0], 49).t().contiguous()


@ops.captures_precision
class StemFn(Function):
    @staticmethod
    def forward(ctx, x, w, b, lnw, lnb, eps, ps):
        C0 = w.shape[0]
        wt = w.reshape(C0, -1).t().contiguous()
        train = any(ctx.needs_input_grad)
        x = x.contiguous().float()
        y, conv, stats = ops.stem_fwd(x, wt, b, lnw, lnb, eps, ps, save=train)
        if train:
            ctx.save_for_backward(x, conv, stats, lnw)
            ctx.ps = ps
            ctx.wshape = tuple(w.shape)
        return y

    @staticmethod
    def backward(ctx, dy):
        x, conv, stats, lnw = ctx.saved_tensors
        dy = dy.contiguous()
        C0 = lnw.shape[0]
        T = conv.numel() // C0
        dlnw, dlnb = _zeros_like_param(lnw), _zeros_like_param(lnw)
        du = ops.layernorm_bwd(dy, conv, stats, lnw, dlnw, dlnb, tokens=T, C=C0)
        N, Cin, H, W = x.shape
        ps = ctx.ps
        K = Cin * ps * ps
        Kp = (K + 31) // 32 * 32
        if C0 % 8 == 0:
            col, _, _ = ops.im2col(x, N=N, H=H, W=W, Cin=Cin, ks=ps, stride=ps, pad=0, Kp=Kp, nchw=True)
            dw2 = torch.zeros((C0, Kp), device=x.device, dtype=torch.float32)
            ops.linear_wgrad(du, col, dw2)
            db = torch.zeros((C0,), device=x.device, dtype=torch.float32)
            ops.colsum(du, db, rows=T, Cc=C0)
            dw = dw2[:, :K].reshape(C0, ps, ps, Cin).permute(0, 3, 1, 2).contiguous()
            return None, dw, db, dlnw, dlnb, None, None
        dwt = torch.zeros((K, C0), device=x.device, dtype=torch.float32)
        db = torch.zeros((C0,), device=x.device, dtype=torch.float32)
        ops.stem_wgrad(x, du, dwt, db, ctx.ps)
        dw = dwt.t().reshape(ctx.wshape).contiguous()
        return None, dw, db, dlnw, dlnb, None, None


@ops.captures_precision
class DownsampleFn(Function):
    @staticmethod
    def forward(ctx, x, lnw, lnb, w, b, eps):
        N, H, W, C = x.shape
        Co = w.shape[0]
        T = N * H * W
        train = any(ctx.needs_input_grad)
        xn = torch.empty((T // 4, 4 * C), device=x.device, dtype=torch.float32)
        _, stats = ops.layernorm_fwd(x, lnw, lnb, eps, tokens=T, C=C, out=xn, out_mode=LN_PATCH2, H=H, W=W,
                                     save_stats=train)
        w2 = w.permute(0, 2, 3, 1).reshape(Co, 4 * C).contiguous()
        y = ops.linear_fwd(xn, w2, b, packed=ops.pack_weight(w2, transposed=False))
        if train:
            ctx.save_for_backward(x, stats, xn, lnw, w2)
            ctx.dims = (N, H, W, C, Co)
        return y.view(N, H // 2, W // 2, Co)

    @staticmethod
    def backward(ctx, dy):
        x, stats, xn, lnw, w2 = ctx.saved_tensors
        N, H, W, C, Co = ctx.dims
        T = N * H * W
        dy2 = dy.contiguous().view(T // 4, Co)
        dxn = ops.linear_dgrad(dy2, w2, packed=ops.pack_weight(w2, transposed=True))
        dw2 = torch.zeros_like(w2)
        ops.linear_wgrad(dy2, xn, dw2)
        db = torch.zeros((Co,), device=x.device, dtype=torch.float32)
        ops.colsum(dy2, db, rows=T // 4, Cc=Co)
        dlnw, dlnb = _zeros_like_param(lnw), _zeros_like_param(lnw)
        dx = ops.layernorm_bwd(dxn, x, stats, lnw, dlnw, dlnb, tokens=T, C=C, in_mode=LN_PATCH2, H=H, W=W)
        dw = dw2.view(Co, 2, 2, C).permute(0, 3, 1, 2).contiguous()
        return dx.view(N, H, W, C), dlnw, dlnb, dw, db, None


@ops.captures_precision
class OutNormFn(Function):
    @staticmethod
    def forward(ctx, x, w, b, eps):
        N, H, W, C = x.shape
        T = N * H * W
        train = any(ctx.needs_input_grad)
        y = torch.empty((N, C, H, W), device=x.device, dtype=torch.float32)
        _, stats = ops.layernorm_fwd(x, w, b, eps, tokens=T, C=C, out=y, out_mode=LN_NCHW, H=H, W=W, save_stats=train)
        if train:
            ctx.save_for_backward(x, stats, w)
        return y

    @staticmethod
    def backward(ctx, dy):
        x, stats, w = ctx.saved_tensors
        N, H, W, C = x.shape
        dw, db = _zeros_like_param(w), _zeros_like_param(w)
        dx = ops.layernorm_bwd(dy.contiguous(), x, stats, w, dw, db, tokens=N * H * W, C=C, in_mode=LN_NCHW, H=H, W=W)
        return dx.view(N, H, W, C), dw, db, None


def _block_front(x, dww, dwb, lnw, lnb, eps, train):
    N, H, W, C = x.shape
    u = ops.dwconv7(x, _taps(dww), dwb)
    v, stats = ops.layernorm_fwd(u, lnw, lnb, eps, tokens=N * H * W, C=C, save_stats=train)
    return u, v.view(N * H * W, C), stats


def _block_front_bwd(dv, dout, x, u, stats, dww, lnw):
    N, H, W, C = x.shape
    T = N * H * W
    dlnw, dlnb = _zeros_like_param(lnw), _zeros_like_param(lnw)
    du = ops.layernorm_bwd(dv, u, stats, lnw, dlnw, dlnb, tokens=T, C=C).view(N, H, W, C)
    dx = ops.dwconv7(du, _taps_flipped(dww), None, resid=dout)
    ddwt = torch.zeros((49, C), device=x.device, dtype=torch.float32)
    ddwb = torch.zeros((C,), device=x.device, dtype=torch.float32)
    ops.dwconv7_wgrad(x, du, ddwt, ddwb)
    ddww = ddwt.t().reshape(C, 1, 7, 7).contiguous()
    return dx, ddww, ddwb, dlnw, dlnb


@ops.captures_precision
class DenseBlockFn(Function):

    @staticmethod
    def forward(ctx, x, dww, dwb, lnw, lnb, w1, b1, w2, b2, gamma, row_scale, eps, packs):
        N, H, W, C = x.shape
        T = N * H * W
        train = any(ctx.needs_input_grad) and packs.get('grad', True)
        fused = packs.get('fused')
        ctx.shortcut = packs.get('shortcut', True)
        resid = x.view(T, C) if ctx.shortcut else None
        if fused is not None:
            u = ops.dwconv7(x, _taps(dww), dwb)
            v_img, v, stats = ops.layernorm_fwd_img(u, lnw, lnb, eps, tokens=T, C=C, save_stats=train, want_f32=train)
            res = ops.ffn_fused_fwd(v_img, packs['w1_c'][0], packs['w2_n'][0], b1, b2, T=T, C=C, chunk=fused['fwd'],
                                    gamma=gamma, row_scale=row_scale, resid=resid, want_aux=train, want_h=train)
            if train:
                ctx.save_for_backward(x, u, stats, v, res[2], res[1], dww, lnw, w1, w2, gamma, row_scale)
                ctx.packs = packs
            return res[0].view(N, H, W, C)
        u, v, stats = _block_front(x, dww, dwb, lnw, lnb, eps, train)
        h = ops.linear_fwd(v, w1, b1, packed=packs.get('w1'))
        a_k, _, _ = ops.act_pack(h, rows=T, width=4 * C, mode=ops.ACT_GELU, want_k=True)
        y2 = torch.empty((T, C), device=x.device, dtype=torch.float32) if train else None
        epi = (EPI_COLSCALE | (EPI_RESID if resid is not None else 0) | (EPI_ROWSCALE if row_scale is not None else 0)
               | (EPI_AUXSTORE if train else 0))
        out = ops.linear_fwd(None, w2, b2, rows=T, a_packed=a_k, epilogue=epi, aux_out=y2, col_scale=gamma,
                             row_scale=row_scale, resid=resid, packed=packs.get('w2'))
        if train:
            ctx.save_for_backward(x, u, stats, v, h, y2, dww, lnw, w1, w2, gamma, row_scale)
            ctx.packs = packs
        return out.view(N, H, W, C)

    @staticmethod
    def backward(ctx, dout):
        x, u, stats, v, h, y2, dww, lnw, w1, w2, gamma, rs = ctx.saved_tensors
        N, H, W, C = x.shape
        T = N * H * W
        dout = dout.contiguous()
        dz = dout.view(T, C)
        dev = x.device
        if rs is None:
            csum, dgamma = ops.colstat(dz, rows=T, Cc=C, y=y2)
        else:
            dgamma = torch.zeros((C,), device=dev, dtype=torch.float32)
            ops.colsum(dz, dgamma, rows=T, Cc=C, b=y2, row_scale=rs)
            csum = torch.zeros((C,), device=dev, dtype=torch.float32)
            ops.colsum(dz, csum, rows=T, Cc=C, row_scale=rs)
        db2 = csum * gamma
        w2g = ops.scale_rows(w2, row_scale=gamma)
        da = ops.linear_dgrad(dz, w2g, epilogue=(EPI_ROWSCALE if rs is not None else 0), row_scale=rs,
                              packed=ops.pack_weight(w2g, transposed=True))
        db1 = torch.zeros((4 * C,), device=dev, dtype=torch.float32)
        dh_k, dh_mn, a_mn = ops.act_pack(h, rows=T, width=4 * C, mode=ops.ACT_BWD, da=da, want_k=True, mn_tile=128,
                                      mn_tile2=ops._pick_bn(4 * C), colsum=db1)
        del da
        dzs = dz if rs is None else ops.scale_rows(dz, row_scale=rs)
        dw2 = torch.zeros_like(w2)
        ops.linear_wgrad(dzs, None, dw2, rows=T, row_scale=gamma, x_packed=a_mn)
        del a_mn
        dw1 = torch.zeros_like(w1)
        ops.linear_wgrad(None, v, dw1, rows=T, dy_packed=dh_mn)
        dv = ops.linear_dgrad(None, w1, rows=T, a_packed=dh_k, packed=ctx.packs.get('w1_t'))
        dx, ddww, ddwb, dlnw, dlnb = _block_front_bwd(dv, dout if ctx.shortcut else None, x, u, stats, dww, lnw)
        return dx, ddww, ddwb, dlnw, dlnb, dw1, db1, dw2, db2, dgamma, None, None, None


def stack_expert_params(params):
    base = params[0]
    step = base.numel() * base.element_size()
    if all(p.is_contiguous() and p.data_ptr() == base.data_ptr() + i * step for i, p in enumerate(params)):
        return
    with torch.no_grad():
        flat = torch.stack([p.data for p in params]).contiguous()
        for i, p in enumerate(params):
            p.data = flat[i]


@ops.captures_precision
class MoEBlockFn(Function):

    @staticmethod
    def forward(ctx, x, dww, dwb, lnw, lnb, gamma, wp, bp, sim, tau, w_noise, row_scale, noise, eps, E, k, record, packs,
                *experts):
        N, H, W, C = x.shape
        T = N * H * W
        w1s, b1s, w2s, b2s = experts[0:E], experts[E:2 * E], experts[2 * E:3 * E], experts[3 * E:4 * E]
        train = any(ctx.needs_input_grad)
        u, v, stats = _block_front(x, dww, dwb, lnw, lnb, eps, train)
        r = ops.moe_router(v, wp, bp, sim, tau, T=T, Cc=C, E=E, k=k, w_noise=w_noise, noise=noise, save=train)
        plan = ops.moe_plan(r['partials'], T=T, E=E, k=k)
        slot_of, pair_token = ops.moe_assign(r['top_idx'], plan, T=T, E=E, k=k)
        R = plan['max_rows']
        grouped = (plan['tile_group'], plan['num_m_tiles'])
        h = ops.linear_fwd(v, w1s[0], b1s[0], row_index=pair_token, rows=R, grouped=grouped, w_group_stride=4 * C * C,
                           bias_group_stride=4 * C, packed=packs.get('w1'))
        a_k, _, _ = ops.act_pack(h, rows=R, width=4 * C, mode=ops.ACT_GELU, want_k=True, live_tiles=plan['num_m_tiles'])
        o = ops.linear_fwd(None, w2s[0], b2s[0], rows=R, a_packed=a_k, grouped=grouped, w_group_stride=4 * C * C,
                           bias_group_stride=C, packed=packs.get('w2'))
        ctx.shortcut = packs.get('shortcut', True)
        out, y = ops.moe_combine(o, slot_of, r['top_idx'], r['top_gate'], gamma, x.view(T, C) if ctx.shortcut else None,
                                 row_scale, T=T, Cc=C, k=k, want_y=record is not None)
        if record is not None:
            record.append(dict(v=v, top_idx=r['top_idx'], top_gate=r['top_gate'], importance=plan['importance'],
                               load=plan['load'], loss=plan['loss'], y=y, counts=plan['counts']))
        if train:
            ctx.noisy = noise is not None
            ctx.save_for_backward(x, u, stats, v, h, o, dww, lnw, gamma, wp, sim, tau, row_scale, r['top_idx'],
                                  r['top_gate'], r['logits'], r['p'], slot_of, pair_token, plan['importance'],
                                  plan['seg_begin'], plan['seg_end'], plan['tile_group'], plan['num_m_tiles'],
                                  w1s[0], w2s[0], noise, r['sigma'], r['top_vals'], r['top_idx_m'], plan['load'],
                                  w_noise)
            ctx.E, ctx.k, ctx.R = E, k, R
            ctx.packs = packs
            ctx.has_noise_param = w_noise is not None
        return out.view(N, H, W, C), plan['loss'].reshape(())

    @staticmethod
    def backward(ctx, dout, dloss):
        (x, u, stats, v, h, o, dww, lnw, gamma, wp, sim, tau, rs, top_idx, top_gate, logits, p, slot_of, pair_token,
         importance, seg_begin, seg_end, tile_group, num_m_tiles, w1, w2, noise, sigma, top_vals, top_idx_m, load,
         w_noise) = ctx.saved_tensors
        E, k, R = ctx.E, ctx.k, ctx.R
        N, H, W, C = x.shape
        T = N * H * W
        dev = x.device
        dout = dout.contiguous()
        dz = dout.view(T, C)
        grouped = (tile_group, num_m_tiles)
        segs = (seg_begin, seg_end)
        d_o = torch.zeros((R, C), device=dev, dtype=torch.float32)
        dgamma = torch.zeros((C,), device=dev, dtype=torch.float32)
        dgate = ops.moe_combine_bwd(dz, o, slot_of, top_idx, top_gate, gamma, rs, d_o, dgamma, T=T, Cc=C, k=k)
        da = ops.linear_dgrad(d_o, w2, grouped=grouped, w_group_stride=4 * C * C, packed=ctx.packs.get('w2_t'))
        db1s = torch.zeros((E, 4 * C), device=dev, dtype=torch.float32)
        dh_k, dh_mn, a_mn = ops.act_pack(h, rows=R, width=4 * C, mode=ops.ACT_BWD, da=da, want_k=True, mn_tile=128,
                                      mn_tile2=ops._pick_bn(4 * C), colsum=db1s, live_tiles=num_m_tiles, tile_group=tile_group)
        del da
        dw2s = torch.zeros((E, C, 4 * C), device=dev, dtype=torch.float32)
        ops.linear_wgrad(d_o, None, dw2s, rows=R, segs=segs, num_groups=E, x_packed=a_mn)
        del a_mn
        db2s = torch.zeros((E, C), device=dev, dtype=torch.float32)
        ops.colsum(d_o, db2s, rows=R, Cc=C, segs=segs, groups=E)
        dw1s = torch.zeros((E, 4 * C, C), device=dev, dtype=torch.float32)
        ops.linear_wgrad(None, v, dw1s, rows=R, x_row_index=pair_token, segs=segs, num_groups=E, dy_packed=dh_mn)
        dxp = torch.empty((R, C), device=dev, dtype=torch.float32)
        ops.linear_dgrad(None, w1, rows=R, a_packed=dh_k, out=dxp, grouped=grouped, w_group_stride=4 * C * C,
                         packed=ctx.packs.get('w1_t'))
        P = wp.shape[0]
        dtau = torch.zeros((1,), device=dev, dtype=torch.float32)
        dsim = torch.zeros((P, E), device=dev, dtype=torch.float32)
        lscale = dloss.reshape(1).contiguous().float()
        noisy = dict(noise=noise, sigma=sigma, top_vals=top_vals, top_idx_m=top_idx_m, load=load) if ctx.noisy else None
        dp, dr = ops.moe_router_bwd(p, sim, tau, top_idx, top_gate, dgate, logits, importance, lscale, dsim, dtau, T=T,
                                    E=E, k=k, noisy=noisy)
        dwp = torch.zeros_like(wp)
        ops.linear_wgrad(dp, v, dwp)
        dbp = torch.zeros((P,), device=dev, dtype=torch.float32)
        ops.colsum(dp, dbp, rows=T, Cc=P)
        dv_r = ops.linear_dgrad(dp, wp, packed=ctx.packs.get('wp_t'))
        dwn = None
        if ctx.noisy:
            wn_t = torch.zeros((32, C), device=dev, dtype=torch.float32)
            wn_t[:E] = w_noise.t()
            dwn_t = torch.zeros((32, C), device=dev, dtype=torch.float32)
            ops.linear_wgrad(dr, v, dwn_t)
            dwn = dwn_t[:E].t().contiguous()
            dv_r = ops.linear_dgrad(dr, wn_t, epilogue=EPI_RESID, resid=dv_r)
        dv = ops.gather_sum(dxp, slot_of, dv_r, T=T, Cc=C, k=k)
        dx, ddww, ddwb, dlnw, dlnb = _block_front_bwd(dv, dout if ctx.shortcut else None, x, u, stats, dww, lnw)
        if dwn is None and ctx.has_noise_param:
            dwn = torch.zeros((C, E), device=dev, dtype=torch.float32)
        grads_e = [dw1s[e] for e in range(E)] + [db1s[e] for e in range(E)] + [dw2s[e] for e in range(E)] + \
                  [db2s[e] for e in range(E)]
        return (dx, ddww, ddwb, dlnw, dlnb, dgamma, dwp, dbp, dsim, dtau, dwn, None, None, None, None, None, None, None,
                *grads_e)


@ops.captures_precision
class DAGateFn(Function):

    @staticmethod
    def forward(ctx, y, x, s, row_scale):
        N, H, W, C = y.shape
        y, x = y.contiguous(), x.contiguous()
        hw = H * W
        out = torch.empty_like(x)
        sc = s if row_scale is None else s * row_scale.view(N, hw)[:, :1]
        sc = sc.contiguous()
        for n in range(N):
            ops.affine(y[n].view(hw, C), a1=sc[n], add=x[n].view(hw, C), out=out[n].view(hw, C))
        ctx.save_for_backward(y, sc, s, row_scale)
        return out

    @staticmethod
    def backward(ctx, d):
        y, sc, s, rs = ctx.saved_tensors
        N, H, W, C = y.shape
        hw = H * W
        d = d.contiguous()
        dy = torch.empty_like(y)
        dsc = torch.zeros((N, C), device=y.device, dtype=torch.float32)
        for n in range(N):
            ops.affine(d[n].view(hw, C), a1=sc[n], out=dy[n].view(hw, C))
            ops.colsum(d[n].view(hw, C), dsc[n], rows=hw, Cc=C, b=y[n].view(hw, C))
        ds = dsc if rs is None else dsc * rs.view(N, hw)[:, :1]
        return dy, d, ds, None


@ops.captures_precision
class SampleMeanFn(Function):

    @staticmethod
    def forward(ctx, y):
        N, H, W, C = y.shape
        y = y.contiguous()
        m = torch.zeros((N, C), device=y.device, dtype=torch.float32)
        for n in range(N):
            ops.colsum(y[n].view(H * W, C), m[n], rows=H * W, Cc=C)
        ctx.shape = (N, H, W, C)
        return m / float(H * W)

    @staticmethod
    def backward(ctx, dm):
        N, H, W, C = ctx.shape
        return (dm / float(H * W)).view(N, 1, 1, C).expand(N, H, W, C).contiguous()
```

sm3det_b200/ops.py:

```python
import ctypes as C
import ctypes as _ct
from typing import Optional

import torch

from . import _lib

SCHED_DENSE, SCHED_GROUPED, SCHED_SPLITK = 0, 1, 2
EPI_BIAS, EPI_GELU, EPI_DGELU, EPI_COLSCALE, EPI_ROWSCALE, EPI_RESID, EPI_ATOMIC, EPI_AUXSTORE, EPI_COLSUM = 1, 2, 4, 8, 16, 32, 64, 128, 256
LN_NHWC, LN_PATCH2, LN_NCHW = 0, 1, 2


import contextlib
import threading

_tls = threading.local()


def current_passes() -> int:
    return getattr(_tls, 'passes', 3)


@contextlib.contextmanager
def precision_scope(passes: int):
    if passes not in (1, 3):
        raise ValueError('mma passes must be 3 (fp32-accurate split-bf16) or 1 (bf16 operands)')
    prev = current_passes()
    _tls.passes = passes
    try:
        yield
    finally:
        _tls.passes = prev


def autocast_passes(module=None) -> int:
    import torch as _t
    return 1 if (getattr(module, 'amp', False) or _t.is_autocast_enabled()) else 3


def captures_precision(cls):
    fwd, bwd = cls.forward, cls.backward

    def forward(ctx, *args, **kwargs):
        ctx._mma_passes = current_passes()
        return fwd(ctx, *args, **kwargs)

    def backward(ctx, *grads):
        with precision_scope(ctx._mma_passes):
            return bwd(ctx, *grads)

    cls.forward = staticmethod(forward)
    cls.backward = staticmethod(backward)
    return cls


def _stream():
    return torch.cuda.current_stream().cuda_stream


def _p(t: Optional[torch.Tensor], dtype=torch.float32):
    if t is None:
        return None
    if not t.is_cuda:
        raise RuntimeError('sm3det_b200 ops need CUDA tensors (no CPU fallback exists)')
    if t.dtype != dtype:
        raise TypeError(f'expected {dtype}, got {t.dtype}')
    if not t.is_contiguous():
        raise ValueError('expected a contiguous tensor')
    return t.data_ptr()


def _pi(t):
    return _p(t, torch.int32)


def _pick_bn(n: int) -> int:
    for bn in (128, 96, 64, 32):
        if n % bn == 0:
            return bn
    raise ValueError(f'N={n} has no GEMM tile width (multiple of 32)')


def num_sms() -> int:
    return torch.cuda.get_device_properties(torch.cuda.current_device()).multi_processor_count


def gemm(*, A, a_smn, a_sk, B, b_smn, b_sk, M, N, K, D, ldd, b_group_stride=0, a_row_index=None, b_k_index=None,
         sched=SCHED_DENSE, k_splits=1, num_groups=1, tile_group=None, num_m_tiles=None, seg_begin=None,
         seg_end=None, d_group_stride=0, bias=None, bias_group_stride=0, epilogue=0, aux_out=None, aux_in=None,
         ld_aux=0, col_scale=None, row_scale=None, resid=None, ld_resid=0, tile_n=0, b_packed=None,
         b_packed_group_stride=0, colsum=None, colsum_group_stride=0, a_packed=None):
    lib = _lib.load()
    a = _lib.GemmArgs()
    a.A = _p(A); a.a_stride_mn = a_smn; a.a_stride_k = a_sk
    a.b_packed = None if b_packed is None else _p(b_packed, torch.int16); a.b_packed_group_stride = b_packed_group_stride
    a.a_packed = None if a_packed is None else _p(a_packed, torch.int16)
    a.B = _p(B); a.b_stride_mn = b_smn; a.b_stride_k = b_sk; a.b_group_stride = b_group_stride
    a.a_row_index = _pi(a_row_index); a.b_k_index = _pi(b_k_index)
    a.M, a.N, a.K = M, N, K
    a.tile_n = tile_n; a.sched = sched; a.k_splits = k_splits; a.num_groups = num_groups
    a.tile_group = _pi(tile_group); a.num_m_tiles = _pi(num_m_tiles)
    a.seg_begin = _pi(seg_begin); a.seg_end = _pi(seg_end)
    a.D = _p(D); a.ldd = ldd; a.d_group_stride = d_group_stride
    a.bias = _p(bias); a.bias_group_stride = bias_group_stride
    a.epilogue = epilogue
    a.aux_out = _p(aux_out); a.aux_in = _p(aux_in); a.ld_aux = ld_aux
    a.col_scale = _p(col_scale); a.row_scale = _p(row_scale)
    a.resid = _p(resid); a.ld_resid = ld_resid
    a.colsum = _p(colsum); a.colsum_group_stride = colsum_group_stride
    a.mma_passes = current_passes()
    _lib.check(lib.sm3_gemm(C.byref(a), _stream()), 'sm3_gemm')
    return D


def pack_weight(w, *, transposed: bool, groups: int = 1, out=None, tile: int = 0):
    lib = _lib.load()
    n_, k_ = w.shape[-2], w.shape[-1]
    if transposed:
        N, K, s_mn, s_k = k_, n_, 1, k_
    else:
        N, K, s_mn, s_k = n_, k_, k_, 1
    per = lib.sm3_gemm_packed_elems(N, K)
    if out is None or out.numel() != groups * per:
        out = torch.empty((groups * per,), device=w.device, dtype=torch.int16)
    if tile:
        _lib.check(lib.sm3_gemm_pack_b_tile(_p(w), s_mn, s_k, n_ * k_, groups, N, K, tile, out.data_ptr(), _stream()),
                   'sm3_gemm_pack_b_tile')
    else:
        _lib.check(lib.sm3_gemm_pack_b(_p(w), s_mn, s_k, n_ * k_, groups, N, K, out.data_ptr(), _stream()), 'sm3_gemm_pack_b')
    return out, per


def pack_act(x, *, rows, cols, mn_major, tile=128, row_index=None, ld=None):
    lib = _lib.load()
    n = lib.sm3_gemm_packed_act_elems(rows, cols, 1 if mn_major else 0, tile)
    out = torch.empty((n,), device=x.device, dtype=torch.int16)
    _lib.check(lib.sm3_gemm_pack_act(_p(x), cols if ld is None else ld, _pi(row_index), rows, cols, 1 if mn_major else 0, tile,
                                     out.data_ptr(), _stream()), 'sm3_gemm_pack_act')
    return out


ACT_GELU, ACT_DGELU, ACT_COPY, ACT_BWD = 0, 1, 2, 3


FFN_FWD, FFN_BWD_DX = 0, 1


def ffn_chunk(mode: int, C: int) -> int:
    import os
    if os.environ.get('SM3_FUSED_FFN', '1') == '0':
        return 0
    return int(_lib.load().sm3_ffn_fused_chunk(mode, C))


def _ffn_args(*, T, C, chunk, mode, a1, wa1, b1, a2=None, wa2=None, wb=None):
    a = _lib.FfnArgs()
    a.a1 = _p(a1, torch.int16); a.a2 = None if a2 is None else _p(a2, torch.int16)
    a.wa1 = _p(wa1, torch.int16); a.wa2 = None if wa2 is None else _p(wa2, torch.int16)
    a.wb = None if wb is None else _p(wb, torch.int16)
    a.bias1 = _p(b1)
    a.M, a.C, a.H4, a.chunk, a.mma_passes, a.mode = T, C, 4 * C, chunk, current_passes(), mode
    return a


def ffn_fused_fwd(v_img, w1_img, w2_img, b1, b2, *, T, C, chunk, gamma=None, row_scale=None, resid=None, want_aux=False,
                  want_h=False):
    lib = _lib.load()
    out = torch.empty((T, C), device=b1.device, dtype=torch.float32)
    aux = torch.empty((T, C), device=b1.device, dtype=torch.float32) if want_aux else None
    h = torch.empty((T, 4 * C), device=b1.device, dtype=torch.float32) if want_h else None
    a = _ffn_args(T=T, C=C, chunk=chunk, mode=FFN_FWD, a1=v_img, wa1=w1_img, b1=b1, wb=w2_img)
    a.bias2 = _p(b2); a.col_scale = _p(gamma); a.row_scale = _p(row_scale); a.resid = _p(resid)
    a.out = _p(out); a.aux_out = _p(aux); a.h_out = _p(h)
    _lib.check(lib.sm3_ffn_fused(_ct.byref(a), _stream()), 'sm3_ffn_fused(fwd)')
    return (out, aux, h) if want_h else (out, aux)


def ffn_fused_bwd(v_img, dz_img, w1_img, w2gt_img, w1t_img, b1, *, T, C, chunk):
    lib = _lib.load()
    out = torch.empty((T, C), device=b1.device, dtype=torch.float32)
    a = _ffn_args(T=T, C=C, chunk=chunk, mode=FFN_BWD_DX, a1=v_img, a2=dz_img, wa1=w1_img, wa2=w2gt_img, b1=b1, wb=w1t_img)
    a.out = _p(out)
    _lib.check(lib.sm3_ffn_fused(_ct.byref(a), _stream()), 'sm3_ffn_fused(bwd)')
    return out


def fused_cost(name, *a, **kw):
    T, Cc = kw['T'], kw['C']
    unit = 2.0 * T * Cc * 4 * Cc
    wbytes = 2 * 4.0 * 4 * Cc * Cc
    if name == 'ffn_fused_fwd':
        return 2 * unit, (3 + (1 if kw.get('want_aux') else 0) + (4 if kw.get('want_h') else 0)) * 4.0 * T * Cc + wbytes, (T, Cc, 'fwd')
    return 2 * unit, 3 * 4.0 * T * Cc + 2 * wbytes, (T, Cc, 'bwd-dv')


def act_pack(h, *, rows, width, mode, da=None, want_k=False, mn_tile=0, want_f32=False, colsum=None, live_tiles=None,
             tile_group=None, mn_tile2=0):
    lib = _lib.load()
    dev = h.device
    a = _lib.ActPackArgs()
    pk = pm = of = None
    if want_k:
        pk = torch.empty((lib.sm3_gemm_packed_act_elems(rows, width, 0, 128),), device=dev, dtype=torch.int16)
    if mn_tile:
        pm = torch.empty((lib.sm3_gemm_packed_act_elems(rows, width, 1, mn_tile),), device=dev, dtype=torch.int16)
    if want_f32:
        of = torch.empty((rows, width), device=dev, dtype=torch.float32)
    a.h = _p(h); a.da = _p(da); a.R = rows; a.W = width; a.mode = mode
    a.live_tiles = _pi(live_tiles); a.tile_group = _pi(tile_group)
    a.out_f32 = _p(of); a.pack_k = None if pk is None else pk.data_ptr(); a.pack_mn = None if pm is None else pm.data_ptr()
    a.mn_tile = mn_tile; a.colsum = _p(colsum)
    pm2 = None
    if mode == ACT_BWD:
        pm2 = torch.empty((lib.sm3_gemm_packed_act_elems(rows, width, 1, mn_tile2),), device=dev, dtype=torch.int16)
        a.pack_mn2 = pm2.data_ptr(); a.mn_tile2 = mn_tile2
    _lib.check(lib.sm3_act_pack(C.byref(a), _stream()), 'sm3_act_pack')
    if mode == ACT_BWD:
        return pk, pm, pm2
    return pk, pm, of


import os as _os
PACK_A_MIN_K = int(_os.environ.get('SM3_PACK_A_MIN_K', '96'))
PACK_W_MIN_TILES = int(_os.environ.get('SM3_PACK_W_MIN_TILES', '2'))


def _pack_a_pays(N, K):
    return K >= PACK_A_MIN_K and (N // _pick_bn(N)) >= 2 or K >= 4 * PACK_A_MIN_K


def linear_fwd(x, w, bias=None, *, epilogue=0, out=None, aux_out=None, col_scale=None, row_scale=None, resid=None,
               row_index=None, rows=None, grouped=None, w_group_stride=0, bias_group_stride=0, packed=None,
               a_packed=None):
    K = w.shape[-1]
    N = w.shape[-2]
    M = rows if rows is not None else x.shape[0]
    if out is None:
        out = torch.empty((M, N), device=w.device, dtype=torch.float32)
    epi = epilogue | (EPI_BIAS if bias is not None else 0)
    kw = {}
    if grouped is not None:
        kw = dict(sched=SCHED_GROUPED, tile_group=grouped[0], num_m_tiles=grouped[1])
    if packed is not None:
        kw.update(b_packed=packed[0], b_packed_group_stride=packed[1])
        if a_packed is not None:
            kw.update(a_packed=a_packed)
            row_index = None
        elif _pack_a_pays(N, K):
            kw.update(a_packed=pack_act(x, rows=M, cols=K, mn_major=False, row_index=row_index))
            row_index = None
    gemm(A=x, a_smn=K, a_sk=1, B=w, b_smn=K, b_sk=1, b_group_stride=w_group_stride, M=M, N=N, K=K, D=out, ldd=N,
         a_row_index=row_index, bias=bias, bias_group_stride=bias_group_stride, epilogue=epi, aux_out=aux_out,
         ld_aux=N, col_scale=col_scale, row_scale=row_scale, resid=resid, ld_resid=N, **kw)
    return out


def linear_dgrad(dy, w, *, epilogue=0, out=None, aux_in=None, row_scale=None, resid=None, grouped=None,
                 w_group_stride=0, packed=None, colsum=None, colsum_group_stride=0, a_packed=None, rows=None):
    N = w.shape[-2]
    M = rows if rows is not None else dy.shape[0]
    K = w.shape[-1]
    if out is None:
        out = torch.empty((M, K), device=w.device, dtype=torch.float32)
    kw = {}
    if grouped is not None:
        kw = dict(sched=SCHED_GROUPED, tile_group=grouped[0], num_m_tiles=grouped[1])
    if packed is not None:
        kw.update(b_packed=packed[0], b_packed_group_stride=packed[1])
        if a_packed is not None:
            kw.update(a_packed=a_packed)
        elif _pack_a_pays(K, N):
            kw.update(a_packed=pack_act(dy, rows=M, cols=N, mn_major=False))
    gemm(A=dy, a_smn=N, a_sk=1, B=w, b_smn=1, b_sk=K, b_group_stride=w_group_stride, M=M, N=K, K=N, D=out, ldd=K,
         epilogue=epilogue | (EPI_COLSUM if colsum is not None else 0), aux_in=aux_in, ld_aux=K, row_scale=row_scale,
         resid=resid, ld_resid=K, colsum=colsum, colsum_group_stride=colsum_group_stride, **kw)
    return out


def linear_wgrad(dy, x, dw, *, rows=None, x_row_index=None, row_scale=None, segs=None, num_groups=1, dy_packed=None,
                 x_packed=None):
    R = rows if rows is not None else dy.shape[0]
    N = dw.shape[-2]
    K = dw.shape[-1]
    tiles = ((N + 127) // 128) * (K // _pick_bn(K)) * num_groups
    splits = -(-3 * num_sms() // max(1, tiles))
    splits = max(1, min(64 if tiles > 1 else 2 * num_sms(), splits, max(1, (R // num_groups) // 1024)))
    epi = EPI_ATOMIC | (EPI_ROWSCALE if row_scale is not None else 0)
    kw = {}
    if dy_packed is not None or x_packed is not None or ((N + 127) // 128) * (K // _pick_bn(K)) >= PACK_W_MIN_TILES:
        if dy_packed is None:
            dy_packed = pack_act(dy, rows=R, cols=N, mn_major=True, tile=128)
        if x_packed is None:
            x_packed = pack_act(x, rows=R, cols=K, mn_major=True, tile=_pick_bn(K), row_index=x_row_index)
        kw = dict(a_packed=dy_packed, b_packed=x_packed)
        x_row_index = None
    gemm(A=dy, a_smn=1, a_sk=N, B=x, b_smn=1, b_sk=K, M=N, N=K, K=R, D=dw, ldd=K, d_group_stride=N * K,
         b_k_index=x_row_index, **kw, sched=SCHED_SPLITK, k_splits=splits, num_groups=num_groups,
         seg_begin=None if segs is None else segs[0], seg_end=None if segs is None else segs[1],
         epilogue=epi, row_scale=row_scale)
    return dw


def layernorm_fwd(x, w, b, eps, *, tokens, C, out=None, out_mode=LN_NHWC, H=0, W=0, save_stats=False):
    lib = _lib.load()
    if out is None:
        out = torch.empty_like(x)
    stats = torch.empty((tokens, 2), device=x.device, dtype=torch.float32) if save_stats else None
    _lib.check(lib.sm3_layernorm_fwd(_p(x), _p(w), _p(b), _p(out), _p(stats), tokens, C, float(eps), out_mode, H, W,
                                     _stream()), 'sm3_layernorm_fwd')
    return out, stats


def layernorm_fwd_img(x, w, b, eps, *, tokens, C, save_stats=False, want_f32=False):
    lib = _lib.load()
    img = torch.empty((lib.sm3_gemm_packed_act_elems(tokens, C, 0, 128),), device=x.device, dtype=torch.int16)
    y = torch.empty((tokens, C), device=x.device, dtype=torch.float32) if want_f32 else None
    stats = torch.empty((tokens, 2), device=x.device, dtype=torch.float32) if save_stats else None
    _lib.check(lib.sm3_layernorm_fwd_img(_p(x), _p(w), _p(b), img.data_ptr(), _p(y), _p(stats), tokens, C, float(eps), _stream()),
               'sm3_layernorm_fwd_img')
    return img, y, stats


def layernorm_bwd(dy, x, stats, w, dw, db, *, tokens, C, in_mode=LN_NHWC, H=0, W=0, dx=None, accumulate=False):
    lib = _lib.load()
    if dx is None:
        dx = torch.empty((tokens, C), device=x.device, dtype=torch.float32)
    _lib.check(lib.sm3_layernorm_bwd(_p(dy), _p(x), _p(stats), _p(w), _p(dx), _p(dw), _p(db), tokens, C, in_mode, H, W,
                                     1 if accumulate else 0, _stream()), 'sm3_layernorm_bwd')
    return dx


def stem_fwd(x, wt, bias, lnw, lnb, eps, ps, *, save=False):
    lib = _lib.load()
    N, Cin, H, W = x.shape
    C0 = wt.shape[1]
    y = torch.empty((N, H // ps, W // ps, C0), device=x.device, dtype=torch.float32)
    conv = torch.empty_like(y) if save else None
    stats = torch.empty((N * (H // ps) * (W // ps), 2), device=x.device, dtype=torch.float32) if save else None
    _lib.check(lib.sm3_stem_fwd(_p(x), _p(wt), _p(bias), _p(lnw), _p(lnb), _p(y), _p(conv), _p(stats), N, Cin, H, W,
                                ps, C0, float(eps), _stream()), 'sm3_stem_fwd')
    return y, conv, stats


def stem_wgrad(x, du, dwt, dbias, ps):
    lib = _lib.load()
    N, Cin, H, W = x.shape
    _lib.check(lib.sm3_stem_wgrad(_p(x), _p(du), _p(dwt), _p(dbias), N, Cin, H, W, ps, dwt.shape[1], _stream()),
               'sm3_stem_wgrad')


def dwconv7(x, wt, bias=None, resid=None, out=None):
    lib = _lib.load()
    N, H, W, Cc = x.shape
    if out is None:
        out = torch.empty_like(x)
    _lib.check(lib.sm3_dwconv7_fwd(_p(x), _p(wt), _p(bias), _p(resid), _p(out), N, H, W, Cc, _stream()), 'sm3_dwconv7_fwd')
    return out


def dwconv7_wgrad(x, dy, dwt, dbias):
    lib = _lib.load()
    N, H, W, Cc = x.shape
    _lib.check(lib.sm3_dwconv7_wgrad(_p(x), _p(dy), _p(dwt), _p(dbias), N, H, W, Cc, _stream()), 'sm3_dwconv7_wgrad')


def moe_router(v, wp, bp, sim, tau, *, T, Cc, E, k, w_noise=None, noise=None, save=False):
    lib = _lib.load()
    P = wp.shape[0]
    dev = v.device
    a = _lib.RouterArgs()
    top_idx = torch.empty((T, k), device=dev, dtype=torch.int32)
    top_gate = torch.empty((T, k), device=dev, dtype=torch.float32)
    logits = torch.empty((T, E), device=dev, dtype=torch.float32) if save else None
    p_out = torch.empty((T, P), device=dev, dtype=torch.float32) if save else None
    m = min(k + 1, E)
    noisy_save = save and noise is not None
    top_vals = torch.empty((T, m), device=dev, dtype=torch.float32) if noisy_save else None
    top_idx_m = torch.empty((T, m), device=dev, dtype=torch.int32) if noisy_save else None
    sigma = torch.empty((T, E), device=dev, dtype=torch.float32) if noisy_save else None
    nb = lib.sm3_moe_router_blocks(T)
    partials = torch.empty((nb, 3 * E), device=dev, dtype=torch.float32)
    a.v = _p(v); a.proj_weight = _p(wp); a.proj_bias = _p(bp); a.sim_matrix = _p(sim); a.temperature = _p(tau)
    a.w_noise = _p(w_noise) if noise is not None else None
    a.noise = _p(noise)
    a.T, a.C, a.P, a.E, a.k = T, Cc, P, E, k
    a.top_idx = _pi(top_idx); a.top_gate = _p(top_gate); a.logits = _p(logits); a.top_vals = _p(top_vals)
    a.p_out = _p(p_out); a.partials = _p(partials); a.sigma = _p(sigma); a.top_idx_m = _pi(top_idx_m)
    _lib.check(lib.sm3_moe_router(C.byref(a), _stream()), 'sm3_moe_router')
    return dict(top_idx=top_idx, top_gate=top_gate, logits=logits, p=p_out, top_vals=top_vals, partials=partials,
                sigma=sigma, top_idx_m=top_idx_m)


def moe_plan(partials, *, T, E, k):
    lib = _lib.load()
    dev = partials.device
    max_tiles = (T * k + 127) // 128 + E
    f = torch.empty(2 * E + 1, device=dev, dtype=torch.float32)
    i = torch.empty(4 * E + max_tiles + 1, device=dev, dtype=torch.int32)
    importance, load, loss = f[:E], f[E:2 * E], f[2 * E:2 * E + 1]
    counts, seg_begin, seg_end, cursor = i[:E], i[E:2 * E], i[2 * E:3 * E], i[3 * E:4 * E]
    tile_group = i[4 * E:4 * E + max_tiles]
    num_m_tiles = i[4 * E + max_tiles:]
    a = _lib.PlanArgs()
    a.partials = _p(partials); a.T, a.E, a.k, a.max_m_tiles = T, E, k, max_tiles
    a.importance = importance.data_ptr(); a.load = load.data_ptr(); a.loss = loss.data_ptr()
    a.counts = counts.data_ptr(); a.seg_begin = seg_begin.data_ptr(); a.seg_end = seg_end.data_ptr()
    a.cursor = cursor.data_ptr(); a.tile_group = tile_group.data_ptr(); a.num_m_tiles = num_m_tiles.data_ptr()
    _lib.check(lib.sm3_moe_plan(C.byref(a), _stream()), 'sm3_moe_plan')
    return dict(importance=importance, load=load, loss=loss, counts=counts, seg_begin=seg_begin, seg_end=seg_end,
                cursor=cursor, tile_group=tile_group, num_m_tiles=num_m_tiles, max_rows=max_tiles * 128)


def moe_assign(top_idx, plan, *, T, E, k):
    lib = _lib.load()
    dev = top_idx.device
    slot_of = torch.empty((T, k), device=dev, dtype=torch.int32)
    pair_token = torch.full((plan['max_rows'],), -1, device=dev, dtype=torch.int32)
    _lib.check(lib.sm3_moe_assign(_pi(top_idx), T, k, E, plan['seg_begin'].data_ptr(), plan['cursor'].data_ptr(),
                                  _pi(slot_of), _pi(pair_token), _stream()), 'sm3_moe_assign')
    return slot_of, pair_token


def moe_combine(o, slot_of, top_idx, gate, gamma, resid, row_scale, *, T, Cc, k, want_y=False):
    lib = _lib.load()
    out = torch.empty((T, Cc), device=o.device, dtype=torch.float32)
    y = torch.empty((T, Cc), device=o.device, dtype=torch.float32) if want_y else None
    _lib.check(lib.sm3_moe_combine(_p(o), _pi(slot_of), _pi(top_idx), _p(gate), _p(gamma), _p(resid), _p(row_scale),
                                   _p(out), _p(y), T, Cc, k, _stream()), 'sm3_moe_combine')
    return out, y


def moe_combine_bwd(dout, o, slot_of, top_idx, gate, gamma, row_scale, d_o, dgamma, *, T, Cc, k):
    lib = _lib.load()
    dgate = torch.empty((T, k), device=o.device, dtype=torch.float32)
    _lib.check(lib.sm3_moe_combine_bwd(_p(dout), _p(o), _pi(slot_of), _pi(top_idx), _p(gate), _p(gamma), _p(row_scale),
                                       _p(d_o), _p(dgate), _p(dgamma), T, Cc, k, _stream()), 'sm3_moe_combine_bwd')
    return dgate


def moe_router_bwd(p, sim, tau, top_idx, top_gate, dgate, logits, importance, loss_scale, dsim, dtau, *, T, E, k,
                   noisy=None):
    lib = _lib.load()
    P = p.shape[1]
    dp = torch.empty_like(p)
    dr = None
    dsim_hat = torch.zeros((P, E), device=p.device, dtype=torch.float32)
    a = _lib.RouterBwdArgs()
    a.p = _p(p); a.sim_matrix = _p(sim); a.temperature = _p(tau); a.top_idx = _pi(top_idx); a.top_gate = _p(top_gate)
    a.dgate = _p(dgate); a.logits = _p(logits); a.importance = importance.data_ptr(); a.loss_scale = _p(loss_scale)
    a.T, a.P, a.E, a.k = T, P, E, k
    a.dp = _p(dp); a.dsim_hat = _p(dsim_hat); a.dtemperature = _p(dtau)
    if noisy is not None:
        dr = torch.empty((T, 32), device=p.device, dtype=torch.float32)
        a.noise = _p(noisy['noise']); a.sigma = _p(noisy['sigma']); a.top_vals = _p(noisy['top_vals'])
        a.top_idx_m = _pi(noisy['top_idx_m']); a.load = noisy['load'].data_ptr(); a.dr = _p(dr)
    _lib.check(lib.sm3_moe_router_bwd(C.byref(a), _stream()), 'sm3_moe_router_bwd')
    _lib.check(lib.sm3_moe_router_bwd_finalize(_p(dsim_hat), _p(sim), _p(dsim), P, E, _stream()),
               'sm3_moe_router_bwd_finalize')
    return dp, dr


def colsum(a, out, *, rows, Cc, b=None, row_scale=None, segs=None, groups=1):
    lib = _lib.load()
    _lib.check(lib.sm3_colsum(_p(a), _p(b), _p(row_scale), None if segs is None else segs[0].data_ptr(),
                              None if segs is None else segs[1].data_ptr(), groups, _p(out), rows, Cc, _stream()),
               'sm3_colsum')
    return out


def gather_sum(src, slot_of, add, *, T, Cc, k, out=None):
    lib = _lib.load()
    if out is None:
        out = torch.empty((T, Cc), device=src.device, dtype=torch.float32)
    _lib.check(lib.sm3_gather_sum(_p(src), _pi(slot_of), _p(add), _p(out), T, Cc, k, _stream()), 'sm3_gather_sum')
    return out


def scale_rows(x, row_scale=None, col_scale=None, out=None):
    lib = _lib.load()
    Cc = x.shape[-1]
    rows = x.numel() // Cc
    if out is None:
        out = torch.empty_like(x)
    _lib.check(lib.sm3_scale_rows(_p(x), _p(row_scale), _p(col_scale), _p(out), rows, Cc, _stream()), 'sm3_scale_rows')
    return out


def dwconv(x, wt, bias=None, resid=None, *, ks, dil=1, out=None):
    lib = _lib.load()
    N, H, W, Cc = x.shape
    if out is None:
        out = torch.empty_like(x)
    _lib.check(lib.sm3_dwconv_fwd(_p(x), _p(wt), _p(bias), _p(resid), _p(out), N, H, W, Cc, ks, dil, _stream()), 'sm3_dwconv_fwd')
    return out


def dwconv_wgrad(x, dy, dwt, dbias, *, ks, dil=1):
    lib = _lib.load()
    N, H, W, Cc = x.shape
    _lib.check(lib.sm3_dwconv_wgrad(_p(x), _p(dy), _p(dwt), _p(dbias), N, H, W, Cc, ks, dil, _stream()), 'sm3_dwconv_wgrad')


def colstat(x, *, rows, Cc, sh1=None, y=None, sh2=None, sc2=None, want_s1=True, want_s2=True):
    lib = _lib.load()
    s = torch.zeros((2, Cc), device=x.device, dtype=torch.float32)
    _lib.check(lib.sm3_colstat(_p(x), _p(sh1), _p(y), _p(sh2), _p(sc2), s[0].data_ptr() if want_s1 else None,
                               s[1].data_ptr() if want_s2 else None, rows, Cc, _stream()), 'sm3_colstat')
    return s[0], s[1]


def affine(x1, a1=None, x2=None, a2=None, b=None, add=None, out=None):
    lib = _lib.load()
    Cc = x1.shape[-1]
    rows = x1.numel() // Cc
    if out is None:
        out = torch.empty_like(x1)
    _lib.check(lib.sm3_affine(_p(x1), _p(a1), _p(x2), _p(a2), _p(b), _p(add), _p(out), rows, Cc, _stream()), 'sm3_affine')
    return out


def mul(a, b, add=None, out=None):
    lib = _lib.load()
    if out is None:
        out = torch.empty_like(a)
    _lib.check(lib.sm3_mul(_p(a), _p(b), _p(add), _p(out), a.numel(), _stream()), 'sm3_mul')
    return out


def dropout(x, p, seed):
    lib = _lib.load()
    out = torch.empty_like(x)
    if torch.is_tensor(seed):
        assert seed.is_cuda and seed.dtype == torch.int64 and seed.numel() == 1
        _lib.check(lib.sm3_dropout_dev(_p(x), _p(out), x.numel(), float(p), seed.data_ptr(), _stream()), 'sm3_dropout_dev')
    else:
        _lib.check(lib.sm3_dropout(_p(x), _p(out), x.numel(), float(p), int(seed), _stream()), 'sm3_dropout')
    return out


def lsk_agg(a1, a2, *, T, Ch, want_idx=True):
    lib = _lib.load()
    agg = torch.empty((T, 2), device=a1.device, dtype=torch.float32)
    amax = torch.empty((T,), device=a1.device, dtype=torch.int32) if want_idx else None
    _lib.check(lib.sm3_lsk_agg(_p(a1), _p(a2), _p(agg), _pi(amax), T, Ch, _stream()), 'sm3_lsk_agg')
    return agg, amax


def conv7_c2(x, w, b, *, N, H, W, act):
    lib = _lib.load()
    y = torch.empty((N * H * W, 2), device=x.device, dtype=torch.float32)
    _lib.check(lib.sm3_conv7_c2(_p(x), _p(w), _p(b), _p(y), N, H, W, act, _stream()), 'sm3_conv7_c2')
    return y


def conv7_c2_wgrad(x, dpre, dw, db, *, N, H, W):
    lib = _lib.load()
    _lib.check(lib.sm3_conv7_c2_wgrad(_p(x), _p(dpre), _p(dw), _p(db), N, H, W, _stream()), 'sm3_conv7_c2_wgrad')


def lsk_mix(a1, a2, sig, *, T, Ch):
    lib = _lib.load()
    out = torch.empty((T, Ch), device=a1.device, dtype=torch.float32)
    _lib.check(lib.sm3_lsk_mix(_p(a1), _p(a2), _p(sig), _p(out), T, Ch, _stream()), 'sm3_lsk_mix')
    return out


def lsk_mix_bwd_sig(dout, a1, a2, sig, *, T, Ch):
    lib = _lib.load()
    dpre = torch.empty((T, 2), device=a1.device, dtype=torch.float32)
    _lib.check(lib.sm3_lsk_mix_bwd_sig(_p(dout), _p(a1), _p(a2), _p(sig), _p(dpre), T, Ch, _stream()), 'sm3_lsk_mix_bwd_sig')
    return dpre


def lsk_mix_bwd_in(dout, sig, dagg, amax, *, T, Ch):
    lib = _lib.load()
    da1 = torch.empty((T, Ch), device=dout.device, dtype=torch.float32)
    da2 = torch.empty((T, Ch), device=dout.device, dtype=torch.float32)
    _lib.check(lib.sm3_lsk_mix_bwd_in(_p(dout), _p(sig), _p(dagg), _pi(amax), _p(da1), _p(da2), T, Ch, _stream()),
               'sm3_lsk_mix_bwd_in')
    return da1, da2


def im2col(x, *, N, H, W, Cin, ks, stride, pad, Kp, nchw):
    lib = _lib.load()
    Ho, Wo = (H + 2 * pad - ks) // stride + 1, (W + 2 * pad - ks) // stride + 1
    col = torch.empty((N * Ho * Wo, Kp), device=x.device, dtype=torch.float32)
    _lib.check(lib.sm3_im2col(_p(x), _p(col), N, H, W, Cin, ks, stride, pad, Kp, 1 if nchw else 0, _stream()), 'sm3_im2col')
    return col, Ho, Wo


def col2im(dcol, *, N, H, W, Cin, ks, stride, pad, Kp, nchw=False):
    lib = _lib.load()
    dx = torch.empty((N, Cin, H, W) if nchw else (N, H, W, Cin), device=dcol.device, dtype=torch.float32)
    _lib.check(lib.sm3_col2im(_p(dcol), _p(dx), N, H, W, Cin, ks, stride, pad, Kp, 1 if nchw else 0, _stream()), 'sm3_col2im')
    return dx


def gather_rows_peer(bases, src_rank, src_row, *, rows, Cc, token_lists=None, scale=None, out=None):
    lib = _lib.load()
    if out is None:
        out = torch.empty((rows, Cc), device=src_rank.device, dtype=torch.float32)
    _lib.check(lib.sm3_gather_rows_peer(_p(bases, torch.int64), None if token_lists is None else _p(token_lists, torch.int64),
                                        _pi(src_rank), _pi(src_row), _p(scale), _p(out), rows, Cc, _stream()),
               'sm3_gather_rows_peer')
    return out


def upsample_add(a, b):
    lib = _lib.load()
    N, H, W, Cc = a.shape
    out = torch.empty_like(a)
    _lib.check(lib.sm3_upsample_add(_p(a), _p(b), _p(out), N, H, W, b.shape[1], b.shape[2], Cc, _stream()), 'sm3_upsample_add')
    return out


def upsample_add_bwd(d, h, w):
    lib = _lib.load()
    N, H, W, Cc = d.shape
    db = torch.empty((N, h, w, Cc), device=d.device, dtype=torch.float32)
    _lib.check(lib.sm3_upsample_add_bwd(_p(d), _p(db), N, H, W, h, w, Cc, _stream()), 'sm3_upsample_add_bwd')
    return db


def transpose_batched(x, B, R, Cc, out_shape):
    lib = _lib.load()
    out = torch.empty(out_shape, device=x.device, dtype=torch.float32)
    _lib.check(lib.sm3_transpose_batched(_p(x), _p(out), B, R, Cc, _stream()), 'sm3_transpose_batched')
    return out
```

Measured before the change: 99.25.

## Fuse FFN backward chain: recompute or load hidden, emit wgrad operands and bias grad

Routes the ConvNeXt-style FFN backward through the fused chain kernel. The kernel either recomputes the hidden pre-activation from the packed LN output (skipping the saved fp32 h when shared memory allows) or loads h from global in a new mode. It also emits the MN-major packed dh and GELU(h) operands for the two weight-gradient GEMMs and reduces db1 into shared memory. This aims to remove the separate dgrad GEMM, activation-pack passes and colsum, and the forward writing of the T×4C hidden tensor. The cost is extra shared memory (act2 and colsum buffers), a workgroup barrier and global copy-out inside the chunk loop, and atomics for db1.

```diff
diff --git a/include/sm3det_b200.h b/include/sm3det_b200.h
--- a/include/sm3det_b200.h
+++ b/include/sm3det_b200.h
@@ -81,8 +81,13 @@
   float* aux_out;
   float* h_out;
   int32_t M, C, H4, chunk, mma_passes, mode;
+  const float* h_in;
+  uint16_t* dh_mn;
+  uint16_t* a_mn;
+  float* colsum;
 } sm3_ffn_args;
 int32_t sm3_ffn_fused_chunk(int32_t mode, int32_t C);
+int32_t sm3_ffn_fused_bwd_needs_h(int32_t C);
 int sm3_ffn_fused(const sm3_ffn_args* args, void* stream);
 size_t sm3_ffn_fused_workspace_bytes(const sm3_ffn_args* args);
 
diff --git a/sm3det_b200/_lib.py b/sm3det_b200/_lib.py
--- a/sm3det_b200/_lib.py
+++ b/sm3det_b200/_lib.py
@@ -58,6 +58,7 @@
         ('out', c_f32p), ('aux_out', c_f32p), ('h_out', c_f32p),
         ('M', C.c_int32), ('C', C.c_int32), ('H4', C.c_int32), ('chunk', C.c_int32), ('mma_passes', C.c_int32),
         ('mode', C.c_int32),
+        ('h_in', c_f32p), ('dh_mn', C.c_void_p), ('a_mn', C.c_void_p), ('colsum', c_f32p),
     ]
 
 
@@ -84,6 +85,7 @@
     'sm3_gemm_pack_b_tile': [_P, _I64, _I64, _I64, _I32, _I32, _I32, _I32, _P, _P],
     'sm3_gemm_workspace_bytes': [C.POINTER(GemmArgs)],
     'sm3_ffn_fused_chunk': [_I32, _I32],
+    'sm3_ffn_fused_bwd_needs_h': [_I32],
     'sm3_ffn_fused': [C.POINTER(FfnArgs), _P],
     'sm3_ffn_fused_workspace_bytes': [C.POINTER(FfnArgs)],
     'sm3_moe_router_workspace_bytes': [C.POINTER(RouterArgs)],
diff --git a/sm3det_b200/backbone.py b/sm3det_b200/backbone.py
--- a/sm3det_b200/backbone.py
+++ b/sm3det_b200/backbone.py
@@ -166,11 +166,18 @@
             w1, w2 = f.pointwise_conv1.weight, f.pointwise_conv2.weight
             C = w2.shape[0]
             cf = ops.ffn_chunk(0, C)
+            cb = ops.ffn_chunk(1, C) if grad and cf > 0 else 0
             if cf > 0:
                 packs = {'fused': dict(fwd=cf), 'w1_c': pc.get('w1', [w1], False, tile=cf), 'w2_n': pc.get('w2', [w2], False, tile=C)}
             else:
                 packs = {'w1': pc.get('w1', [w1], False), 'w2': pc.get('w2', [w2], False)}
-            if grad:
+            if cb > 0:
+                needs_h = ops.ffn_bwd_needs_h(C)
+                packs['fused'].update(bwd=cb, needs_h=needs_h)
+                if not needs_h:
+                    packs['w1_cb'] = pc.get('w1', [w1], False, tile=cb)
+                packs['w1_tn'] = pc.get('w1', [w1], True, tile=C)
+            elif grad:
                 packs['w1_t'] = pc.get('w1', [w1], True)
             packs['grad'] = grad
             packs['shortcut'] = shortcut
diff --git a/sm3det_b200/csrc/capi.cu b/sm3det_b200/csrc/capi.cu
--- a/sm3det_b200/csrc/capi.cu
+++ b/sm3det_b200/csrc/capi.cu
@@ -63,7 +63,8 @@
 }
 size_t sm3_gemm_workspace_bytes(const sm3_gemm_args*) { return 0; }
 
-int32_t sm3_ffn_fused_chunk(int32_t mode, int32_t C) { return (mode == 0 || mode == 1) ? ffn::chain_chunk(mode, C) : 0; }
+int32_t sm3_ffn_fused_chunk(int32_t mode, int32_t C) { return mode == 0 ? ffn::chain_chunk(0, C) : mode == 1 ? ffn::chain_bwd_chunk(C) : 0; }
+int32_t sm3_ffn_fused_bwd_needs_h(int32_t C) { return ffn::chain_bwd_needs_h(C); }
 size_t sm3_ffn_fused_workspace_bytes(const sm3_ffn_args*) { return 0; }
 int sm3_ffn_fused(const sm3_ffn_args* a, void* stream) {
   if (!a) { set_last_error("sm3_ffn_fused: null args"); return SM3_ERR_INVALID_ARG; }
@@ -72,6 +73,7 @@
   p.bias1 = a->bias1; p.bias2 = a->bias2; p.col_scale = a->col_scale; p.row_scale = a->row_scale; p.resid = a->resid;
   p.out = a->out; p.aux_out = a->aux_out; p.h_out = a->h_out;
   p.M = a->M; p.C = a->C; p.H4 = a->H4; p.HC = a->chunk; p.passes = a->mma_passes; p.mode = a->mode;
+  p.h_in = a->h_in; p.dh_mn = a->dh_mn; p.a_mn = a->a_mn; p.colsum = a->colsum;
   return ffn::chain(p, S(stream));
 }
 
diff --git a/sm3det_b200/csrc/ffn_fused.cu b/sm3det_b200/csrc/ffn_fused.cu
--- a/sm3det_b200/csrc/ffn_fused.cu
+++ b/sm3det_b200/csrc/ffn_fused.cu
@@ -15,7 +15,7 @@
 constexpr uint32_t BARS = 256;
 
 struct Layout {
-  uint32_t a, ones, a2, wa, wb, act, act2, stage, bar, total;
+  uint32_t a, ones, a2, wa, wb, act, act2, cs, stage, bar, total;
   uint32_t a_tile, wa_chunk, wa_stage, wb_stage, act_bytes;
   int sa, sb;
 };
@@ -67,12 +67,17 @@
   auto wb_empty = [&](int s) { return bar + 64u + 8u * s; };
   const int warp = threadIdx.x >> 5, lane = threadIdx.x & 31;
   constexpr int NA = (MODE == 1) ? 2 : 1;
+  const uint16_t* a_first = MODE == 2 ? p.a2 : p.a1;
+  const uint16_t* wa_first = MODE == 2 ? p.wa2 : p.wa1;
+  const bool emit = MODE != 0 && (p.dh_mn || p.a_mn);
 
   if (threadIdx.x == 0) {
     mbar_init(a_full, 1); mbar_init(a_empty, NE);
     for (int s = 0; s < 2; ++s) { mbar_init(wa_full(s), 1); mbar_init(wa_empty(s), NE); mbar_init(wb_full(s), 1); mbar_init(wb_empty(s), NE); }
     asm volatile("fence.mbarrier_init.release.cluster;" ::: "memory");
   }
+  if (MODE != 0 && p.colsum)
+    for (int c = threadIdx.x; c < p.H4; c += THREADS) asm volatile("st.shared.f32 [%0], %1;" ::"r"(sb0 + L.cs + 4u * c), "f"(0.f) : "memory");
   __syncthreads();
   const int nch = k.nch;
   constexpr int kbc = C / 32;
@@ -85,7 +90,7 @@
         mbar_wait(a_empty, (n_t & 1u) ^ 1u);
         if ((p.debug & 8) && n_t > 0) { mbar_arrive(a_full); goto weights; }
         expect_tx(a_full, NA * L.a_tile);
-        bulk_g2s(sb0 + L.a, reinterpret_cast<const uint8_t*>(p.a1) + (long long)t * L.a_tile, L.a_tile, a_full);
+        bulk_g2s(sb0 + L.a, reinterpret_cast<const uint8_t*>(a_first) + (long long)t * L.a_tile, L.a_tile, a_full);
         if (MODE == 1) bulk_g2s(sb0 + L.a + L.a_tile, reinterpret_cast<const uint8_t*>(p.a2) + (long long)t * L.a_tile, L.a_tile, a_full);
       weights:
         for (int j = 0; j < nch; ++j, ++n_w) {
@@ -94,7 +99,7 @@
           if ((p.debug & 4) && n_w >= (uint32_t)L.sa) { mbar_arrive(wa_full(s)); continue; }
           expect_tx(wa_full(s), L.wa_stage);
           const uint32_t dst = sb0 + L.wa + s * L.wa_stage;
-          bulk_g2s(dst, reinterpret_cast<const uint8_t*>(p.wa1) + (long long)j * L.wa_chunk, L.wa_chunk, wa_full(s));
+          bulk_g2s(dst, reinterpret_cast<const uint8_t*>(wa_first) + (long long)j * L.wa_chunk, L.wa_chunk, wa_full(s));
           if (MODE == 1) bulk_g2s(dst + L.wa_chunk, reinterpret_cast<const uint8_t*>(p.wa2) + (long long)j * L.wa_chunk, L.wa_chunk, wa_full(s));
         }
       }
@@ -128,7 +133,7 @@
       for (int q = 0; q < NA; ++q) {
         uint64_t da = make_smem_desc(sb0 + L.a + q * L.a_tile + slab, false), db = make_smem_desc(wst + q * L.wa_chunk, false);
         for (int kb = 0; kb < kbc; ++kb) {
-          if (q == 0) {
+          if (MODE != 2 && q == 0) {
             mma3<HC>(acc_h, da, da + 512u, db, db + HC * 4u, kb > 0 ? 1u : 0u, p.passes);
             mma3<HC>(acc_h, da + 2u, da + 514u, db + 2u, db + HC * 4u + 2u, 1u, p.passes);
           } else {
@@ -139,7 +144,49 @@
         }
       }
     };
+    auto load_h = [&](int t, int j) {
+#pragma unroll
+      for (int q = 0; q < HC / 8; ++q)
+#pragma unroll
+        for (int h = 0; h < 2; ++h) {
+          const long long row = (long long)t * 128 + r_lo + 8 * h;
+          const float2 x = row < p.M ? __ldg(reinterpret_cast<const float2*>(p.h_in + row * p.H4 + (long long)j * HC + 8 * q + 2 * (lane & 3)))
+                                     : make_float2(0.f, 0.f);
+          acc_h[4 * q + 2 * h] = x.x; acc_h[4 * q + 2 * h + 1] = x.y;
+        }
+    };
+    const long long kb_mn = (p.M + 31) / 32;
+    auto copy_out = [&](int t, int j) {
+      constexpr int CPR = HC / 8;
+      const int mt = (j * HC) >> 7;
+      const uint32_t mc0 = (uint32_t)((j * HC) & 127) >> 3;
+      const int tid = threadIdx.x - (EPI0 + 4 * g) * 32;
+#pragma unroll
+      for (int u = tid; u < 64 * CPR; u += 128) {
+        const int r = u / CPR, c = u % CPR;
+        const long long kb = ((long long)t * 128 + g * 64 + r) >> 5;
+        if (kb >= kb_mn) continue;
+        const uint32_t so = (uint32_t)(c >> 2) * 16384u + kmajor_sw64_offset((uint32_t)(g * 64 + r), (uint32_t)(c & 3));
+        const long long go = ((long long)mt * kb_mn + kb) * 16384LL + mnmajor_sw128_offset((uint32_t)(r & 31), mc0 + (uint32_t)c);
+        uint32_t v0, v1, v2, v3;
+        if (p.dh_mn) {
+#pragma unroll
+          for (int pl = 0; pl < 2; ++pl) {
+            asm volatile("ld.shared.v4.b32 {%0, %1, %2, %3}, [%4];" : "=r"(v0), "=r"(v1), "=r"(v2), "=r"(v3) : "r"(sb0 + L.act + so + pl * 8192u));
+            *reinterpret_cast<uint4*>(reinterpret_cast<uint8_t*>(p.dh_mn) + go + pl * 8192) = make_uint4(v0, v1, v2, v3);
+          }
+        }
+        if (p.a_mn) {
+#pragma unroll
+          for (int pl = 0; pl < 2; ++pl) {
+            asm volatile("ld.shared.v4.b32 {%0, %1, %2, %3}, [%4];" : "=r"(v0), "=r"(v1), "=r"(v2), "=r"(v3) : "r"(sb0 + L.act2 + so + pl * 8192u));
+            *reinterpret_cast<uint4*>(reinterpret_cast<uint8_t*>(p.a_mn) + go + pl * 8192) = make_uint4(v0, v1, v2, v3);
+          }
+        }
+      }
+    };
     for (int t = blockIdx.x; t < k.m_tiles; t += gridDim.x, ++n_t) {
+      if constexpr (MODE == 2) load_h(t, 0);
       mbar_wait(a_full, n_t & 1u);
       wg::fence();
       gemm_a(n_c);
@@ -147,18 +194,20 @@
       for (int j = 0; j < nch; ++j, ++n_c) {
         wg::wait<0>();
         wg::fence_operand(acc_h);
-        if constexpr (MODE == 1) wg::fence_operand(acc_d);
+        if constexpr (MODE != 0) wg::fence_operand(acc_d);
         __syncwarp();
         if (lane == 0) {
           mbar_arrive(wa_empty(n_c % L.sa));
           if (j > 0) mbar_arrive(wb_empty((n_b - 1) % L.sb));
           if (j == nch - 1) mbar_arrive(a_empty);
         }
+        if (emit) wg_bar();
         const float* b1 = p.bias1 + (long long)j * HC;
 #pragma unroll
         for (int q = 0; q < HC / 8; ++q) {
           const int kk = 8 * q + 2 * (lane & 3);
-          const float2 bv = __ldg(reinterpret_cast<const float2*>(b1 + kk));
+          const float2 bv = MODE == 2 ? make_float2(0.f, 0.f) : __ldg(reinterpret_cast<const float2*>(b1 + kk));
+          float cs0 = 0.f, cs1 = 0.f;
 #pragma unroll
           for (int h = 0; h < 2; ++h) {
             const int r = r_lo + 8 * h;
@@ -168,16 +217,42 @@
               if (row < p.M) *reinterpret_cast<float2*>(p.h_out + row * p.H4 + (long long)j * HC + kk) = make_float2(x0, x1);
             }
             float y0, y1;
+            const uint32_t o = sb0 + L.act + (uint32_t)(kk >> 5) * 16384u + kmajor_sw64_offset((uint32_t)r, (uint32_t)((kk & 31) >> 3)) +
+                               (uint32_t)(kk & 7) * 2u;
             if (p.debug & 1) { y0 = x0; y1 = x1; }
             else if constexpr (MODE == 0) { y0 = gelu_fast(x0); y1 = gelu_fast(x1); }
-            else { y0 = acc_d[4 * q + 2 * h] * gelu_grad_fast(x0); y1 = acc_d[4 * q + 2 * h + 1] * gelu_grad_fast(x1); }
+            else {
+              const bool live = (long long)t * 128 + r < p.M;
+              float P0, e0, P1, e1;
+              phi_parts(x0, P0, e0);
+              phi_parts(x1, P1, e1);
+              y0 = live ? acc_d[4 * q + 2 * h] * fmaf(x0 * 0.39894228040143267794f, e0, P0) : 0.f;
+              y1 = live ? acc_d[4 * q + 2 * h + 1] * fmaf(x1 * 0.39894228040143267794f, e1, P1) : 0.f;
+              cs0 += y0; cs1 += y1;
+              if (p.a_mn) {
+                uint32_t hi, lo;
+                split2(live ? x0 * P0 : 0.f, live ? x1 * P1 : 0.f, hi, lo);
+                asm volatile("st.shared.b32 [%0], %1;" ::"r"(o - L.act + L.act2), "r"(hi) : "memory");
+                asm volatile("st.shared.b32 [%0], %1;" ::"r"(o - L.act + L.act2 + 8192u), "r"(lo) : "memory");
+              }
+            }
             if (p.debug & 2) continue;
             uint32_t hi, lo;
             split2(y0, y1, hi, lo);
-            const uint32_t o = sb0 + L.act + (uint32_t)(kk >> 5) * 16384u + kmajor_sw64_offset((uint32_t)r, (uint32_t)((kk & 31) >> 3)) +
-                               (uint32_t)(kk & 7) * 2u;
             asm volatile("st.shared.b32 [%0], %1;" ::"r"(o), "r"(hi) : "memory");
             asm volatile("st.shared.b32 [%0], %1;" ::"r"(o + 8192u), "r"(lo) : "memory");
+          }
+          if (MODE != 0 && p.colsum) {
+#pragma unroll
+            for (int sh = 4; sh < 32; sh <<= 1) {
+              cs0 += __shfl_xor_sync(0xffffffffu, cs0, sh);
+              cs1 += __shfl_xor_sync(0xffffffffu, cs1, sh);
+            }
+            if (lane < 4) {
+              const uint32_t ca = sb0 + L.cs + 4u * (uint32_t)(j * HC + kk);
+              asm volatile("red.shared.add.f32 [%0], %1;" ::"r"(ca), "f"(cs0) : "memory");
+              asm volatile("red.shared.add.f32 [%0], %1;" ::"r"(ca + 4u), "f"(cs1) : "memory");
+            }
           }
         }
         fence_proxy_async_smem();
@@ -198,6 +273,8 @@
         ++n_b;
         if (j + 1 < nch) gemm_a(n_c + 1);
         wg::commit();
+        if constexpr (MODE == 2) { if (j + 1 < nch) load_h(t, j + 1); }
+        if (emit) copy_out(t, j);
       }
       wg::wait<0>();
       wg::fence_operand(acc_o);
@@ -242,11 +319,19 @@
         }
       }
     }
+    if (MODE != 0 && p.colsum) {
+      asm volatile("bar.sync 3, 256;" ::: "memory");
+      for (int c = threadIdx.x - EPI0 * 32; c < p.H4; c += NE * 32) {
+        float v;
+        asm volatile("ld.shared.f32 %0, [%1];" : "=f"(v) : "r"(sb0 + L.cs + 4u * c) : "memory");
+        atomicAdd(p.colsum + c, v);
+      }
+    }
   }
 }
 
-static bool chain_layout(int mode, int C, int HC, int sa, int sb, Layout& L) {
-  const uint32_t nA = mode == 1 ? 2 : 1;
+static bool chain_layout(int kmode, int C, int HC, int sa, int sb, bool emit, Layout& L) {
+  const uint32_t nA = kmode == 1 ? 2 : 1;
   L.a_tile = (uint32_t)(C / 32) * 16384u;
   L.wa_chunk = (uint32_t)(C / 32) * HC * 128u;
   L.wa_stage = nA * L.wa_chunk;
@@ -259,41 +344,63 @@
   L.wa = o; o += sa * L.wa_stage;
   L.wb = o; o += sb * L.wb_stage;
   L.act = o; o += L.act_bytes;
-  L.act2 = 0;
+  L.act2 = 0; L.cs = 0;
+  if (emit) {
+    L.act2 = o; o += L.act_bytes;
+    L.cs = o; o += (uint32_t)C * 16u;
+  }
   L.stage = o; o += STAGING;
   L.bar = o; o += BARS;
   L.total = o + 1024u;
   return L.total <= SMEM_LIMIT + 1024u;
 }
 
-static bool pick_chain(int mode, int C, int HC_req, int& HC, Layout& L) {
+static bool pick_chain(int kmode, int C, bool emit, int HC_req, int& HC, Layout& L) {
   static const int cand[][3] = {{64, 2, 2}, {32, 2, 2}, {64, 2, 1}, {32, 2, 1}, {32, 1, 1}};
   if (C % 32 != 0 || C < 32 || C > 256) return false;
   for (auto& c : cand)
-    if ((HC_req == 0 || c[0] == HC_req) && chain_layout(mode, C, c[0], c[1], c[2], L)) { HC = c[0]; return true; }
+    if ((HC_req == 0 || c[0] == HC_req) && chain_layout(kmode, C, c[0], c[1], c[2], emit, L)) { HC = c[0]; return true; }
   return false;
+}
+
+int chain_bwd_needs_h(int C) {
+  int HC = 0; Layout L;
+  return pick_chain(1, C, true, 0, HC, L) ? 0 : 1;
 }
 
 int chain_chunk(int mode, int C) {
   int HC = 0; Layout L;
-  return pick_chain(mode, C, 0, HC, L) ? HC : 0;
+  return pick_chain(mode, C, false, 0, HC, L) ? HC : 0;
+}
+
+int chain_bwd_chunk(int C) {
+  int HC = 0; Layout L;
+  return pick_chain(chain_bwd_needs_h(C) ? 2 : 1, C, true, 0, HC, L) ? HC : 0;
 }
 
 static bool aligned16(const void* q) { return (reinterpret_cast<uintptr_t>(q) & 15u) == 0; }
 
 int chain(const ChainParams& p, cudaStream_t stream) {
   SM3_REQUIRE(p.mode == 0 || p.mode == 1, SM3_ERR_INVALID_ARG, "ffn chain: mode");
-  SM3_REQUIRE(p.a1 && p.wa1 && p.wb && p.bias1 && p.out && (p.mode == 0 || (p.a2 && p.wa2)), SM3_ERR_INVALID_ARG, "ffn chain: null operand");
+  const int kmode = (p.mode == 1 && p.h_in) ? 2 : p.mode;
+  const bool emit = p.mode == 1 && (p.dh_mn || p.a_mn || p.colsum);
+  SM3_REQUIRE(p.wb && p.bias1 && p.out && (kmode == 2 || (p.a1 && p.wa1)) && (p.mode == 0 || (p.a2 && p.wa2)), SM3_ERR_INVALID_ARG,
+              "ffn chain: null operand");
   SM3_REQUIRE(p.M > 0 && p.H4 > 0 && p.C > 0, SM3_ERR_INVALID_ARG, "ffn chain: bad shape");
   ChainK k{};
   k.p = p;
   int HC = 0;
   SM3_REQUIRE(p.HC == 32 || p.HC == 64, SM3_ERR_INVALID_ARG, "ffn chain: chunk must be 32 or 64 (sm3_ffn_fused_chunk), got %d", p.HC);
-  SM3_REQUIRE(pick_chain(p.mode, p.C, p.HC, HC, k.L), SM3_ERR_UNSUPPORTED_SHAPE, "ffn chain: C=%d with chunk %d does not fit shared memory (mode %d)", p.C, p.HC, p.mode);
+  SM3_REQUIRE(pick_chain(kmode, p.C, emit, p.HC, HC, k.L), SM3_ERR_UNSUPPORTED_SHAPE,
+              "ffn chain: C=%d with chunk %d does not fit shared memory (mode %d%s)", p.C, p.HC, p.mode,
+              kmode == 1 && emit ? "; this C needs h_in, see sm3_ffn_fused_bwd_needs_h" : "");
   SM3_REQUIRE(p.H4 % HC == 0 && p.C % 16 == 0, SM3_ERR_UNSUPPORTED_SHAPE, "ffn chain: H4=%d not a multiple of the chunk %d", p.H4, HC);
-  SM3_REQUIRE(aligned16(p.a1) && aligned16(p.wa1) && aligned16(p.wb) && aligned16(p.out) && aligned16(p.bias1) &&
+  SM3_REQUIRE(!emit || p.H4 == 4 * p.C, SM3_ERR_UNSUPPORTED_SHAPE, "ffn chain: backward outputs need H4 = 4C, got H4=%d C=%d", p.H4, p.C);
+  SM3_REQUIRE((!p.a1 || aligned16(p.a1)) && (!p.wa1 || aligned16(p.wa1)) && aligned16(p.wb) && aligned16(p.out) && aligned16(p.bias1) &&
               (!p.a2 || aligned16(p.a2)) && (!p.wa2 || aligned16(p.wa2)) && (!p.resid || aligned16(p.resid)) &&
-              (!p.aux_out || aligned16(p.aux_out)) && (!p.bias2 || aligned16(p.bias2)) && (!p.col_scale || aligned16(p.col_scale)),
+              (!p.aux_out || aligned16(p.aux_out)) && (!p.bias2 || aligned16(p.bias2)) && (!p.col_scale || aligned16(p.col_scale)) &&
+              (!p.row_scale || aligned16(p.row_scale)) && (!p.h_out || aligned16(p.h_out)) && (!p.h_in || aligned16(p.h_in)) &&
+              (!p.dh_mn || aligned16(p.dh_mn)) && (!p.a_mn || aligned16(p.a_mn)),
               SM3_ERR_INVALID_ARG, "ffn chain: pointers must be 16B aligned");
   k.p.passes = (p.passes == 1) ? 1 : 3;
   k.m_tiles = (p.M + 127) / 128;
@@ -312,8 +419,9 @@
     case 160: SM3_CHAIN_LAUNCH(MODE_, HC_, 160); break; case 192: SM3_CHAIN_LAUNCH(MODE_, HC_, 192); break;                 \
     case 224: SM3_CHAIN_LAUNCH(MODE_, HC_, 224); break; default: SM3_CHAIN_LAUNCH(MODE_, HC_, 256); break;                  \
   }
-  if (p.mode == 0) { if (HC == 64) { SM3_CHAIN_C(0, 64) } else { SM3_CHAIN_C(0, 32) } }
-  else { if (HC == 64) { SM3_CHAIN_C(1, 64) } else { SM3_CHAIN_C(1, 32) } }
+  if (kmode == 0) { if (HC == 64) { SM3_CHAIN_C(0, 64) } else { SM3_CHAIN_C(0, 32) } }
+  else if (kmode == 1) { if (HC == 64) { SM3_CHAIN_C(1, 64) } else { SM3_CHAIN_C(1, 32) } }
+  else { if (HC == 64) { SM3_CHAIN_C(2, 64) } else { SM3_CHAIN_C(2, 32) } }
 #undef SM3_CHAIN_C
 #undef SM3_CHAIN_LAUNCH
   return check_launch("ffn_chain_kernel");
diff --git a/sm3det_b200/csrc/ffn_fused.cuh b/sm3det_b200/csrc/ffn_fused.cuh
--- a/sm3det_b200/csrc/ffn_fused.cuh
+++ b/sm3det_b200/csrc/ffn_fused.cuh
@@ -21,10 +21,16 @@
   float* h_out;
   int M, C, H4, HC, passes, mode;
   int debug;
+  const float* h_in;
+  uint16_t* dh_mn;
+  uint16_t* a_mn;
+  float* colsum;
 };
 int chain(const ChainParams& p, cudaStream_t stream);
 
 int chain_chunk(int mode, int C);
+int chain_bwd_chunk(int C);
+int chain_bwd_needs_h(int C);
 
 }
 }
diff --git a/sm3det_b200/functional.py b/sm3det_b200/functional.py
--- a/sm3det_b200/functional.py
+++ b/sm3det_b200/functional.py
@@ -150,10 +150,14 @@
         if fused is not None:
             u = ops.dwconv7(x, _taps(dww), dwb)
             v_img, v, stats = ops.layernorm_fwd_img(u, lnw, lnb, eps, tokens=T, C=C, save_stats=train, want_f32=train)
+            fused_bwd = train and fused.get('bwd', 0) > 0
+            want_h = train and (not fused_bwd or fused['needs_h'])
             res = ops.ffn_fused_fwd(v_img, packs['w1_c'][0], packs['w2_n'][0], b1, b2, T=T, C=C, chunk=fused['fwd'],
-                                    gamma=gamma, row_scale=row_scale, resid=resid, want_aux=train, want_h=train)
+                                    gamma=gamma, row_scale=row_scale, resid=resid, want_aux=train, want_h=want_h)
             if train:
-                ctx.save_for_backward(x, u, stats, v, res[2], res[1], dww, lnw, w1, w2, gamma, row_scale)
+                ctx.save_for_backward(x, u, stats, v, res[2] if want_h else None, res[1], dww, lnw, w1, w2, gamma, row_scale,
+                                      b1, v_img if fused_bwd and not want_h else None)
+                ctx.fused_bwd = fused['bwd'] if fused_bwd else 0
                 ctx.packs = packs
             return res[0].view(N, H, W, C)
         u, v, stats = _block_front(x, dww, dwb, lnw, lnb, eps, train)
@@ -165,13 +169,14 @@
         out = ops.linear_fwd(None, w2, b2, rows=T, a_packed=a_k, epilogue=epi, aux_out=y2, col_scale=gamma,
                              row_scale=row_scale, resid=resid, packed=packs.get('w2'))
         if train:
-            ctx.save_for_backward(x, u, stats, v, h, y2, dww, lnw, w1, w2, gamma, row_scale)
+            ctx.save_for_backward(x, u, stats, v, h, y2, dww, lnw, w1, w2, gamma, row_scale, b1, None)
+            ctx.fused_bwd = 0
             ctx.packs = packs
         return out.view(N, H, W, C)
 
     @staticmethod
     def backward(ctx, dout):
-        x, u, stats, v, h, y2, dww, lnw, w1, w2, gamma, rs = ctx.saved_tensors
+        x, u, stats, v, h, y2, dww, lnw, w1, w2, gamma, rs, b1, v_img = ctx.saved_tensors
         N, H, W, C = x.shape
         T = N * H * W
         dout = dout.contiguous()
@@ -186,6 +191,24 @@
             ops.colsum(dz, csum, rows=T, Cc=C, row_scale=rs)
         db2 = csum * gamma
         w2g = ops.scale_rows(w2, row_scale=gamma)
+        if ctx.fused_bwd:
+            cb = ctx.fused_bwd
+            dzs = dz if rs is None else ops.scale_rows(dz, row_scale=rs)
+            dz_img = ops.pack_act(dzs, rows=T, cols=C, mn_major=False)
+            db1 = torch.zeros((4 * C,), device=dev, dtype=torch.float32)
+            w1c = ctx.packs.get('w1_cb')
+            dv, dh_mn, a_mn = ops.ffn_fused_bwd(v_img, dz_img, None if w1c is None else w1c[0],
+                                                ops.pack_weight(w2g, transposed=True, tile=cb)[0], ctx.packs['w1_tn'][0], b1,
+                                                T=T, C=C, chunk=cb, h=h, db1=db1, want_wgrad_operands=True)
+            del dz_img
+            dw2 = torch.zeros_like(w2)
+            ops.linear_wgrad(dzs, None, dw2, rows=T, row_scale=gamma, x_packed=a_mn)
+            del a_mn
+            dw1 = torch.zeros_like(w1)
+            ops.linear_wgrad(None, v, dw1, rows=T, dy_packed=dh_mn)
+            del dh_mn
+            dx, ddww, ddwb, dlnw, dlnb = _block_front_bwd(dv, dout if ctx.shortcut else None, x, u, stats, dww, lnw)
+            return dx, ddww, ddwb, dlnw, dlnb, dw1, db1, dw2, db2, dgamma, None, None, None
         da = ops.linear_dgrad(dz, w2g, epilogue=(EPI_ROWSCALE if rs is not None else 0), row_scale=rs,
                               packed=ops.pack_weight(w2g, transposed=True))
         db1 = torch.zeros((4 * C,), device=dev, dtype=torch.float32)
diff --git a/sm3det_b200/ops.py b/sm3det_b200/ops.py
--- a/sm3det_b200/ops.py
+++ b/sm3det_b200/ops.py
@@ -153,6 +153,10 @@
     return int(_lib.load().sm3_ffn_fused_chunk(mode, C))
 
 
+def ffn_bwd_needs_h(C: int) -> bool:
+    return bool(_lib.load().sm3_ffn_fused_bwd_needs_h(C))
+
+
 def _ffn_args(*, T, C, chunk, mode, a1, wa1, b1, a2=None, wa2=None, wb=None):
     a = _lib.FfnArgs()
     a.a1 = _p(a1, torch.int16); a.a2 = None if a2 is None else _p(a2, torch.int16)
@@ -176,13 +180,23 @@
     return (out, aux, h) if want_h else (out, aux)
 
 
-def ffn_fused_bwd(v_img, dz_img, w1_img, w2gt_img, w1t_img, b1, *, T, C, chunk):
+def ffn_fused_bwd(v_img, dz_img, w1_img, w2gt_img, w1t_img, b1, *, T, C, chunk, h=None, db1=None, want_wgrad_operands=False):
     lib = _lib.load()
     out = torch.empty((T, C), device=b1.device, dtype=torch.float32)
-    a = _ffn_args(T=T, C=C, chunk=chunk, mode=FFN_BWD_DX, a1=v_img, a2=dz_img, wa1=w1_img, wa2=w2gt_img, b1=b1, wb=w1t_img)
-    a.out = _p(out)
+    a = _lib.FfnArgs()
+    a.a1 = None if v_img is None else _p(v_img, torch.int16); a.a2 = _p(dz_img, torch.int16)
+    a.wa1 = None if w1_img is None else _p(w1_img, torch.int16); a.wa2 = _p(w2gt_img, torch.int16)
+    a.wb = _p(w1t_img, torch.int16); a.bias1 = _p(b1)
+    a.M, a.C, a.H4, a.chunk, a.mma_passes, a.mode = T, C, 4 * C, chunk, current_passes(), FFN_BWD_DX
+    a.out = _p(out); a.h_in = _p(h); a.colsum = _p(db1)
+    dh_mn = a_mn = None
+    if want_wgrad_operands:
+        n = lib.sm3_gemm_packed_act_elems(T, 4 * C, 1, 128)
+        dh_mn = torch.empty((n,), device=b1.device, dtype=torch.int16)
+        a_mn = torch.empty((n,), device=b1.device, dtype=torch.int16)
+        a.dh_mn = dh_mn.data_ptr(); a.a_mn = a_mn.data_ptr()
     _lib.check(lib.sm3_ffn_fused(_ct.byref(a), _stream()), 'sm3_ffn_fused(bwd)')
-    return out
+    return (out, dh_mn, a_mn) if want_wgrad_operands else out
 
 
 def fused_cost(name, *a, **kw):
@@ -191,7 +205,8 @@
     wbytes = 2 * 4.0 * 4 * Cc * Cc
     if name == 'ffn_fused_fwd':
         return 2 * unit, (3 + (1 if kw.get('want_aux') else 0) + (4 if kw.get('want_h') else 0)) * 4.0 * T * Cc + wbytes, (T, Cc, 'fwd')
-    return 2 * unit, 3 * 4.0 * T * Cc + 2 * wbytes, (T, Cc, 'bwd-dv')
+    hidden = (4 if kw.get('h') is not None else 0) + (8 if kw.get('want_wgrad_operands') else 0)
+    return 2 * unit, (3 + hidden) * 4.0 * T * Cc + 2 * wbytes, (T, Cc, 'bwd')
 
 
 def act_pack(h, *, rows, width, mode, da=None, want_k=False, mn_tile=0, want_f32=False, colsum=None, live_tiles=None,
```

Result: faster. 100.5, median of 6 (+1.2%).
